# zhoujoey/ORB-SLAM3-Mac

Hardware: AMD Instinct MI355X
Metric: ORB extract+match frames/sec (higher is better)
Workload: dtype u8; 1 GPU; vga: synthetic 640x480 batch=1024 per GPU, 8-level pyramid, 1000 feats/frame, ORB extract + Hamming 2-NN match (Frame.cc:1146) + SearchForInitialization (ORBmatcher.cc:710) vs successor frame; pipelines=1, matchers=side by side (two contexts), frames_total=1024

## Files before the change

include/orbhip.h:

```cpp
#ifndef ORBHIP_H
#define ORBHIP_H
#include <stddef.h>
#include <stdint.h>
#ifdef __cplusplus
extern "C" {
#endif

#define ORBHIP_OK 0
#define ORBHIP_E_BADARG (-1)
#define ORBHIP_E_NODEVICE (-2)
#define ORBHIP_E_HIP (-3)
#define ORBHIP_E_CAPACITY (-4)
#define ORBHIP_E_ABORTED (-5)
#define ORBHIP_E_NOTSPD (-6)
#define ORBHIP_E_EMPTY (-7)

typedef struct {
    float x, y, size, angle, response;
    int32_t octave, class_id;
} orbhip_keypoint;

typedef struct orbhip_ctx orbhip_ctx;
typedef struct orbhip_extractor orbhip_extractor;

const char *orbhip_version(void);
const char *orbhip_last_error(void);

int orbhip_ctx_create(int device, void *stream, orbhip_ctx **out);
void orbhip_ctx_destroy(orbhip_ctx *ctx);
int orbhip_ctx_synchronize(orbhip_ctx *ctx);
int orbhip_ctx_wait_for(orbhip_ctx *ctx, orbhip_ctx *other);
int orbhip_ctx_check_status(orbhip_ctx *ctx);
void *orbhip_ctx_stream(orbhip_ctx *ctx);

int orbhip_extractor_create(orbhip_ctx *ctx, int nfeatures, float scale_factor, int nlevels,
                            int ini_th_fast, int min_th_fast, orbhip_extractor **out);
void orbhip_extractor_destroy(orbhip_extractor *ext);

int orbhip_extractor_levels(const orbhip_extractor *ext);
int orbhip_extractor_table(const orbhip_extractor *ext, int which, float *out);
int orbhip_extractor_features_per_level(const orbhip_extractor *ext, int *out);
int orbhip_extractor_umax(const orbhip_extractor *ext, int *out16);
int orbhip_blur_half_widths(int *out19);

int orbhip_extractor_reserve(orbhip_extractor *ext, int width, int height, int max_batch);
int orbhip_extractor_max_keypoints(const orbhip_extractor *ext);

int orbhip_extract_batch_device(orbhip_extractor *ext, const uint8_t *d_images, int width,
                                int height, size_t row_stride, size_t frame_stride, int batch,
                                int lap0, int lap1);
int orbhip_extractor_results(orbhip_extractor *ext, orbhip_keypoint **d_kp, uint8_t **d_desc,
                             int32_t **d_count, int32_t **d_mono_index);
int orbhip_extract_batch_host(orbhip_extractor *ext, const uint8_t *h_images, int width, int height,
                              size_t row_stride, size_t frame_stride, int batch, int lap0, int lap1,
                              orbhip_keypoint *kp_out, uint8_t *desc_out, int cap,
                              int32_t *count_out, int32_t *mono_out);
int orbhip_extract_batch_host_view(orbhip_extractor *ext, const uint8_t *h_images, int width, int height, size_t row_stride,
                                   size_t frame_stride, int batch, int lap0, int lap1, const orbhip_keypoint **kp_view,
                                   const uint8_t **desc_view, int *row_capacity, const int32_t **count_view, const int32_t **mono_view);
int orbhip_extractor_blur_kernel(const orbhip_extractor *ext, int batch);
int orbhip_extractor_fast_kernel(const orbhip_extractor *ext);
int orbhip_extractor_blur_tiled(const orbhip_extractor *ext, int batch);
int orbhip_extractor_desc_plan(const orbhip_extractor *ext, int batch, int32_t *kp_base, int32_t *kp_cap, int32_t *waves_per_xcd);

int orbhip_extractor_resize_band_rows(const orbhip_extractor *ext, int level);

int orbhip_extractor_last_frame(orbhip_extractor *ext, int frame, const orbhip_keypoint **d_kp, const uint8_t **d_desc,
                                const orbhip_keypoint **h_kp_view, const uint8_t **h_desc_view, int32_t *count, unsigned long long *generation);

int orbhip_extractor_level_dims(const orbhip_extractor *ext, int level, int *w, int *h);
int orbhip_extractor_get_pyramid_level(orbhip_extractor *ext, int frame, int level, int padded,
                                       uint8_t *h_out, size_t out_stride);
int orbhip_extractor_get_pyramid_padded(orbhip_extractor *ext, int frame, uint8_t *const *levels_out, const size_t *strides);
int orbhip_extractor_get_blurred_level(orbhip_extractor *ext, int frame, int level,
                                       uint8_t *h_out, size_t out_stride);
int orbhip_extractor_get_fast_candidates(orbhip_extractor *ext, int frame, int level,
                                         int32_t *xs, int32_t *ys, int32_t *scores, int cap,
                                         int32_t *n_out);
int orbhip_extractor_get_level_keypoints(orbhip_extractor *ext, int frame, int level,
                                         orbhip_keypoint *out, int cap, int32_t *n_out);

int orbhip_extractor_set_graph_mode(orbhip_extractor *ext, int enable);

#define ORBHIP_STAGE_PYRAMID 0
#define ORBHIP_STAGE_FAST_CELLS 1
#define ORBHIP_STAGE_BLUR 2
#define ORBHIP_STAGE_OCTREE 3
#define ORBHIP_STAGE_DESC 4
#define ORBHIP_STAGE_ASSEMBLE 5
#define ORBHIP_STAGE_COUNT 6
int orbhip_extractor_set_profiling(orbhip_extractor *ext, int enable);
int orbhip_extractor_stage_ms(orbhip_extractor *ext, float *ms_out );

int orbhip_descriptor_distance(const uint8_t *a32, const uint8_t *b32);

int orbhip_match_bf2nn_device(orbhip_ctx *ctx, const uint8_t *d_descA, const int32_t *d_nA,
                              size_t strideA, const uint8_t *d_descB, const int32_t *d_nB,
                              size_t strideB, int pairs, int max_n, double ratio,
                              int32_t *d_idx2, int32_t *d_dist2, uint8_t *d_accept);

int orbhip_search_for_initialization_device(orbhip_ctx *ctx,
        const orbhip_keypoint *d_kpA, const uint8_t *d_descA, const int32_t *d_nA,
        const orbhip_keypoint *d_kpB, const uint8_t *d_descB, const int32_t *d_nB,
        int pairs, int max_n, size_t frame_stride_kp , float min_x, float min_y,
        float max_x, float max_y, int window_size, float nn_ratio, int check_orientation,
        float *d_prev_matched, int32_t *d_matches12, int32_t *d_nmatches);

int orbhip_prev_matched_init_device(orbhip_ctx *ctx, const orbhip_keypoint *d_kp, size_t frame_stride_kp,
                                    int frames, int max_n, float *d_prev_matched);

typedef struct orbhip_proj_query {
    float u, v, radius, ur, angle;
    int32_t min_level, max_level, has_obs;
} orbhip_proj_query;
int orbhip_search_by_projection_device(orbhip_ctx *ctx, const orbhip_proj_query *d_q, const uint8_t *d_desc_q,
                                       const int32_t *d_nq, int max_q, const orbhip_keypoint *d_kp,
                                       const uint8_t *d_desc, const float *d_u_right, const int32_t *d_n, int max_n,
                                       size_t frame_stride_kp, int pairs, float min_x, float min_y, float max_x,
                                       float max_y, int th_high, int check_orientation, int32_t *d_train_match,
                                       int32_t *d_nmatches);

int orbhip_search_local_map_device(orbhip_ctx *ctx, const orbhip_proj_query *d_q, const uint8_t *d_desc_q,
                                   const int32_t *d_nq, int max_q, const orbhip_keypoint *d_kp,
                                   const uint8_t *d_desc, const float *d_u_right, const int32_t *d_n, int max_n,
                                   size_t frame_stride_kp, int pairs, float min_x, float min_y, float max_x,
                                   float max_y, int th_high, float nn_ratio, int32_t *d_train_match,
                                   int32_t *d_nmatches);

int orbhip_search_by_projection_rig_device(orbhip_ctx *ctx, int mode, const orbhip_proj_query *d_q, const uint8_t *d_desc_q,
                                           const int32_t *d_nq, int max_q, const orbhip_keypoint *d_kp, const uint8_t *d_desc,
                                           const int32_t *d_n, const int32_t *d_nleft, const int32_t *d_mirror, int max_n,
                                           size_t frame_stride_kp, int pairs, float min_x, float min_y, float max_x, float max_y,
                                           int th_high, float nn_ratio, int check_orientation, int32_t *d_train_match,
                                           int32_t *d_nmatches);

int orbhip_debug_sbp_handed_back(orbhip_ctx *ctx, int32_t *flags_out, int cap, int *pairs_out);

int orbhip_search_by_projection_host(orbhip_ctx *ctx, int mode, const orbhip_proj_query *q, const uint8_t *desc_q, int nq,
                                     const orbhip_keypoint *kp, const uint8_t *desc, const float *u_right, int n,
                                     float min_x, float min_y, float max_x, float max_y, int th_high, float nn_ratio,
                                     int check_orientation, int32_t *train_match_inout, int32_t *nmatches_out);
int orbhip_search_by_projection_rig_host(orbhip_ctx *ctx, int mode, const orbhip_proj_query *q, const uint8_t *desc_q, int nq,
                                         const orbhip_keypoint *kp, const uint8_t *desc, int n, int nleft, const int32_t *mirror,
                                         float min_x, float min_y, float max_x, float max_y, int th_high, float nn_ratio,
                                         int check_orientation, int32_t *train_match_inout, int32_t *nmatches_out);
int orbhip_search_for_initialization_host(orbhip_ctx *ctx, const orbhip_keypoint *kpA, const uint8_t *descA, int nA,
                                          const orbhip_keypoint *kpB, const uint8_t *descB, int nB, float min_x, float min_y,
                                          float max_x, float max_y, int window_size, float nn_ratio, int check_orientation,
                                          float *prev_matched_inout, int32_t *matches12_out, int32_t *nmatches_out);
int orbhip_search_by_projection_host_resident(orbhip_ctx *ctx, int mode, const orbhip_proj_query *q, const uint8_t *desc_q, int nq,
                                              const orbhip_keypoint *kp_host, const orbhip_keypoint *d_kp, const uint8_t *d_desc, const float *u_right, int n,
                                              float min_x, float min_y, float max_x, float max_y, int th_high, float nn_ratio,
                                              int check_orientation, int32_t *train_match_inout, int32_t *nmatches_out);
int orbhip_search_for_initialization_host_resident(orbhip_ctx *ctx, const orbhip_keypoint *kpA, const uint8_t *descA, int nA,
                                                   const orbhip_keypoint *kpB_host, const orbhip_keypoint *d_kpB, const uint8_t *d_descB, int nB, float min_x, float min_y,
                                                   float max_x, float max_y, int window_size, float nn_ratio, int check_orientation,
                                                   float *prev_matched_inout, int32_t *matches12_out, int32_t *nmatches_out);

int orbhip_fuse_search_device(orbhip_ctx *ctx, const orbhip_proj_query *d_q, const uint8_t *d_desc_q, const int32_t *d_nq,
                              int max_q, const orbhip_keypoint *d_kp, const uint8_t *d_desc, const float *d_u_right,
                              const int32_t *d_n, int max_n, size_t frame_stride_kp, int pairs,
                              const float *inv_level_sigma2, int nlevels, float min_x, float min_y, float max_x, float max_y,
                              int32_t *d_best_idx, int32_t *d_best_dist);

int orbhip_search_by_bow_device(orbhip_ctx *ctx,
        const int32_t *d_kf_node_ids, const int32_t *d_kf_node_start, const int32_t *d_kf_feat, const int32_t *d_kf_nnodes,
        const uint8_t *d_kf_valid, const orbhip_keypoint *d_kf_kp, const uint8_t *d_kf_desc,
        const int32_t *d_f_node_ids, const int32_t *d_f_node_start, const int32_t *d_f_feat, const int32_t *d_f_nnodes,
        const orbhip_keypoint *d_f_kp, const uint8_t *d_f_desc, const int32_t *d_nF,
        int pairs, int max_nodes, int max_n, size_t frame_stride_kp, float nn_ratio, int check_orientation,
        int32_t *d_match_f, int32_t *d_nmatches);

int orbhip_search_by_bow_rig_device(orbhip_ctx *ctx,
        const int32_t *d_kf_node_ids, const int32_t *d_kf_node_start, const int32_t *d_kf_feat, const int32_t *d_kf_nnodes,
        const uint8_t *d_kf_valid, const orbhip_keypoint *d_kf_kp, const uint8_t *d_kf_desc,
        const int32_t *d_f_node_ids, const int32_t *d_f_node_start, const int32_t *d_f_feat, const int32_t *d_f_nnodes,
        const orbhip_keypoint *d_f_kp, const uint8_t *d_f_desc, const int32_t *d_nF, const int32_t *d_nleft,
        int pairs, int max_nodes, int max_n, size_t frame_stride_kp, float nn_ratio, int check_orientation,
        int32_t *d_match_f, int32_t *d_nmatches);

int orbhip_search_by_bow_host(orbhip_ctx *ctx,
        const int32_t *kf_node_ids, const int32_t *kf_node_start, const int32_t *kf_feat, int kf_nnodes, const uint8_t *kf_valid,
        const orbhip_keypoint *kf_kp, const uint8_t *kf_desc, int nK,
        const int32_t *f_node_ids, const int32_t *f_node_start, const int32_t *f_feat, int f_nnodes,
        const orbhip_keypoint *f_kp, const uint8_t *f_desc, int nF, int nleft,
        float nn_ratio, int check_orientation, int32_t *match_f_out, int32_t *nmatches_out);
int orbhip_search_by_bow_host_resident(orbhip_ctx *ctx,
        const int32_t *kf_node_ids, const int32_t *kf_node_start, const int32_t *kf_feat, int kf_nnodes, const uint8_t *kf_valid,
        const orbhip_keypoint *kf_kp, const uint8_t *kf_desc, int nK,
        const int32_t *f_node_ids, const int32_t *f_node_start, const int32_t *f_feat, int f_nnodes,
        const orbhip_keypoint *f_kp_host, const orbhip_keypoint *d_f_kp, const uint8_t *d_f_desc, int nF,
        float nn_ratio, int check_orientation, int32_t *match_f_out, int32_t *nmatches_out);

int orbhip_search_by_bow_kf_device(orbhip_ctx *ctx,
        const int32_t *d_node_ids1, const int32_t *d_node_start1, const int32_t *d_feat1, const int32_t *d_nnodes1,
        const uint8_t *d_valid1, const orbhip_keypoint *d_kp1, const uint8_t *d_desc1, const int32_t *d_n1,
        const int32_t *d_node_ids2, const int32_t *d_node_start2, const int32_t *d_feat2, const int32_t *d_nnodes2,
        const uint8_t *d_valid2, const orbhip_keypoint *d_kp2, const uint8_t *d_desc2, const int32_t *d_n2,
        int pairs, int max_nodes, int max_n, size_t frame_stride_kp, float nn_ratio, int check_orientation,
        int32_t *d_matches12, int32_t *d_nmatches);

typedef struct orbhip_tri_pair { float F12[9]; float ep_x, ep_y; int32_t only_stereo, coarse; } orbhip_tri_pair;

int orbhip_search_for_triangulation_device(orbhip_ctx *ctx,
        const int32_t *d_nid1, const uint8_t *d_has_mp1, const orbhip_keypoint *d_kp1, const uint8_t *d_desc1, const float *d_u_right1,
        const int32_t *d_n1,
        const int32_t *d_node_ids2, const int32_t *d_node_start2, const int32_t *d_feat2, const int32_t *d_nnodes2,
        const uint8_t *d_has_mp2, const orbhip_keypoint *d_kp2, const uint8_t *d_desc2, const float *d_u_right2, const int32_t *d_n2,
        const orbhip_tri_pair *d_pair, int pairs, int max_nodes, int max_n, size_t frame_stride_kp,
        const float *scale_factors, const float *level_sigma2, int nlevels, int check_orientation,
        int32_t *d_matches12, int32_t *d_nmatches);

typedef struct orbhip_tri_pair_general {
    float R12[4][9], t12[4][3];
    float F12[4][9];
    float cam1[2][8], cam2[2][8];
    int32_t cam1_type[2], cam2_type[2];
    float ep_x, ep_y;
    int32_t nleft1, nleft2;
    int32_t only_stereo, coarse;
} orbhip_tri_pair_general;
int orbhip_search_for_triangulation_general_device(orbhip_ctx *ctx,
        const int32_t *d_nid1, const uint8_t *d_has_mp1, const orbhip_keypoint *d_kp1, const uint8_t *d_desc1, const float *d_u_right1,
        const int32_t *d_n1,
        const int32_t *d_node_ids2, const int32_t *d_node_start2, const int32_t *d_feat2, const int32_t *d_nnodes2,
        const uint8_t *d_has_mp2, const orbhip_keypoint *d_kp2, const uint8_t *d_desc2, const float *d_u_right2, const int32_t *d_n2,
        const orbhip_tri_pair_general *d_pair, int pairs, int max_nodes, int max_n, size_t frame_stride_kp,
        const float *level_sigma2_1, const float *scale_factors2, const float *level_sigma2_2, int nlevels, int check_orientation,
        int32_t *d_matches12, int32_t *d_nmatches);

typedef struct orbhip_tri_pair_poses { float Tcw1[2][12], Tcw2[2][12]; } orbhip_tri_pair_poses;
int orbhip_match_and_triangulate_device(orbhip_ctx *ctx,
        const int32_t *d_nid1, const uint8_t *d_has_mp1, const orbhip_keypoint *d_kp1, const uint8_t *d_desc1, const int32_t *d_n1,
        const int32_t *d_node_ids2, const int32_t *d_node_start2, const int32_t *d_feat2, const int32_t *d_nnodes2,
        const uint8_t *d_has_mp2, const orbhip_keypoint *d_kp2, const uint8_t *d_desc2, const int32_t *d_n2,
        const orbhip_tri_pair_general *d_pair, const orbhip_tri_pair_poses *d_poses, int pairs, int max_nodes, int max_n, size_t frame_stride_kp,
        const float *level_sigma2_1, const float *level_sigma2_2, int nlevels, int check_orientation,
        int32_t *d_matches12, float *d_points12, int32_t *d_nmatches);
int orbhip_match_and_triangulate_host(orbhip_ctx *ctx,
        const int32_t *nid1, const uint8_t *has_mp1, const orbhip_keypoint *kp1, const uint8_t *desc1, int n1,
        const int32_t *node_ids2, const int32_t *node_start2, const int32_t *feat2, int nnodes2,
        const uint8_t *has_mp2, const orbhip_keypoint *kp2, const uint8_t *desc2, int n2,
        const orbhip_tri_pair_general *pair, const orbhip_tri_pair_poses *poses, const float *level_sigma2_1, const float *level_sigma2_2,
        int nlevels, int check_orientation, int32_t *matches12_out, float *points12_out, int32_t *nmatches_out);

typedef struct orbhip_newpoints_pair {
    float cam1[2][8], cam2[2][8];
    int32_t cam1_type[2], cam2_type[2];
    int32_t nleft1, nleft2;
    float Tcw1[2][12], Tcw2[2][12];
    float Twc1[12], Twc2[12];
    float Ow1[2][3], Ow2[2][3];
    float mb1, mb2;
    float mbf;
    float ratio_factor;
    int32_t far_points;
    float th_far_points;
} orbhip_newpoints_pair;
int orbhip_create_new_map_points_device(orbhip_ctx *ctx,
        const orbhip_keypoint *d_kp1, const orbhip_keypoint *d_kp1_raw, const float *d_u_right1, const float *d_depth1, const int32_t *d_n1,
        const orbhip_keypoint *d_kp2, const orbhip_keypoint *d_kp2_raw, const float *d_u_right2, const float *d_depth2, const int32_t *d_n2,
        const int32_t *d_matches12, const orbhip_newpoints_pair *pair, int pairs, int max_n, size_t frame_stride_kp,
        const float *level_sigma2_1, const float *scale_factors1, const float *level_sigma2_2, const float *scale_factors2, int nlevels,
        uint8_t *d_has_mp1, uint8_t *d_has_mp2, float *d_x3D, uint8_t *d_outcome, int32_t *d_n_created);

typedef struct orbhip_newpoints_keyframe {
    const orbhip_keypoint *kp;
    const orbhip_keypoint *kp_raw;
    const uint8_t *desc;
    const float *u_right, *depth;
    const uint8_t *has_mp;
    int32_t n;
    const int32_t *nid;
    const int32_t *node_ids, *node_start, *feat;
    int32_t nnodes;
    const float *level_sigma2, *scale_factors;
} orbhip_newpoints_keyframe;
int orbhip_create_new_map_points_host(orbhip_ctx *ctx, const orbhip_newpoints_keyframe *cur, const orbhip_newpoints_keyframe *neigh,
        const orbhip_tri_pair_general *geom, const orbhip_newpoints_pair *pair, int n_neigh, int nlevels, int check_orientation,
        int32_t *matches12_out, float *x3D_out, uint8_t *outcome_out, int32_t *n_created_out, uint8_t *has_mp1_out);

int orbhip_search_for_triangulation_host(orbhip_ctx *ctx,
        const int32_t *nid1, const uint8_t *has_mp1, const orbhip_keypoint *kp1, const uint8_t *desc1, const float *u_right1, int n1,
        const int32_t *node_ids2, const int32_t *node_start2, const int32_t *feat2, int nnodes2,
        const uint8_t *has_mp2, const orbhip_keypoint *kp2, const uint8_t *desc2, const float *u_right2, int n2,
        const orbhip_tri_pair_general *pair, const float *level_sigma2_1, const float *scale_factors2, const float *level_sigma2_2,
        int nlevels, int check_orientation, int32_t *matches12_out, int32_t *nmatches_out);
int orbhip_fuse_search_host(orbhip_ctx *ctx, const orbhip_proj_query *q, const uint8_t *desc_q, int nq, const orbhip_keypoint *kp,
                            const uint8_t *desc, const float *u_right, int n, const float *inv_level_sigma2, int nlevels,
                            float min_x, float min_y, float max_x, float max_y, int32_t *best_idx_out, int32_t *best_dist_out);
int orbhip_search_by_bow_kf_host(orbhip_ctx *ctx,
        const int32_t *node_ids1, const int32_t *node_start1, const int32_t *feat1, int nnodes1, const uint8_t *valid1,
        const orbhip_keypoint *kp1, const uint8_t *desc1, int n1,
        const int32_t *node_ids2, const int32_t *node_start2, const int32_t *feat2, int nnodes2, const uint8_t *valid2,
        const orbhip_keypoint *kp2, const uint8_t *desc2, int n2,
        float nn_ratio, int check_orientation, int32_t *matches12_out, int32_t *nmatches_out);

int orbhip_undistort_keypoints_device(orbhip_ctx *ctx, const orbhip_keypoint *d_kp, const int32_t *d_n, int frames, int max_n,
                                      size_t frame_stride_kp, float fx, float fy, float cx, float cy, const float *dist_coef,
                                      int n_dist, orbhip_keypoint *d_kp_un);

int orbhip_assign_features_to_grid_device(orbhip_ctx *ctx, const orbhip_keypoint *d_kp, const int32_t *d_n, int frames, int max_n,
                                          size_t frame_stride_kp, float min_x, float min_y, float max_x, float max_y,
                                          int32_t *d_cell_start, int32_t *d_items);

int orbhip_assign_features_to_grid_rig_device(orbhip_ctx *ctx, const orbhip_keypoint *d_kp, const int32_t *d_n, const int32_t *d_nleft,
                                              int frames, int max_n, size_t frame_stride_kp, float min_x, float min_y, float max_x,
                                              float max_y, int32_t *d_cell_start, int32_t *d_items);

int orbhip_bow_vectors_device(orbhip_ctx *ctx, const int32_t *d_word_id, const double *d_weight, const int32_t *d_node_id,
                              const int32_t *d_n, int frames, int max_n, int max_nodes,
                              int32_t *d_node_ids, int32_t *d_node_start, int32_t *d_feat, int32_t *d_nnodes,
                              int32_t *d_bow_word, double *d_bow_value, int32_t *d_nwords);

int orbhip_distinctive_descriptors_device(orbhip_ctx *ctx, const uint8_t *d_desc, const int32_t *d_n, int points, int max_n,
                                          int32_t *d_best_idx, uint8_t *d_best_desc);

int orbhip_bow_transform_device(orbhip_ctx *ctx, const uint8_t *d_desc, const int32_t *d_n, int frames, int max_n,
                                size_t frame_stride, const uint8_t *d_node_desc, const int32_t *d_child_start,
                                const int32_t *d_child_ids, const int32_t *d_node_word, const double *d_node_weight,
                                int L, int levelsup, int32_t *d_word_id, double *d_weight, int32_t *d_nid);

int orbhip_compute_stereo_matches_device(orbhip_extractor *left, orbhip_extractor *right, float mb, float mbf,
                                         float *d_u_right, float *d_depth, int32_t *d_n_matches);

int orbhip_compute_stereo_matches_host(orbhip_extractor *left, orbhip_extractor *right, float mb, float mbf,
                                       float *u_right_out, float *depth_out, int n, int32_t *n_matches_out);

int orbhip_compute_stereo_fisheye_matches_device(orbhip_ctx *ctx,
        const orbhip_keypoint *d_kpL, const uint8_t *d_descL, const int32_t *d_nL, const int32_t *d_monoL, size_t strideL,
        const orbhip_keypoint *d_kpR, const uint8_t *d_descR, const int32_t *d_nR, const int32_t *d_monoR, size_t strideR,
        int batch, int max_n, int cam1_type, const float *cam1, int cam2_type, const float *cam2, const float *Rlr, const float *tlr,
        const float *level_sigma2, int nlevels,
        int32_t *d_l2r, int32_t *d_r2l, float *d_depth, float *d_x3d, int32_t *d_n_matches);

int orbhip_compute_stereo_fisheye_matches_host(orbhip_extractor *left, orbhip_extractor *right, int cam1_type, const float *cam1,
        int cam2_type, const float *cam2, const float *Rlr, const float *tlr, const float *level_sigma2, int nlevels,
        int32_t *l2r_out, float *depth_out, float *x3d_out, int n_left, int32_t *r2l_out, int n_right, int32_t *n_matches_out);

typedef struct {
    int32_t n_poses;
    int32_t n_points;
    int32_t n_edges;
    const uint8_t *pose_fixed;
    const int32_t *edge_pose;
    const int32_t *edge_point;
// ... 394 lines not shown
```

orb-slam3-mac_amd/csrc/fast_kernels.hip:

```cpp
#include "orb_internal.h"
#include "wave_dpp.h"
#include <algorithm>
#include <mutex>
#include <vector>
#include <cstdio>
#include <cstdlib>
#include <cstring>

typedef short s16x2 __attribute__((ext_vector_type(2)));
typedef uint32_t u32_unaligned __attribute__((aligned(1)));

__device__ __forceinline__ s16x2 as_s16x2(uint32_t v) { return __builtin_bit_cast(s16x2, v); }
__device__ __forceinline__ uint32_t as_u32(s16x2 v) { return __builtin_bit_cast(uint32_t, v); }
__device__ __forceinline__ s16x2 pkmin(s16x2 a, s16x2 b) { return __builtin_elementwise_min(a, b); }
__device__ __forceinline__ s16x2 pkmax(s16x2 a, s16x2 b) { return __builtin_elementwise_max(a, b); }
__device__ __forceinline__ s16x2 pkmin3(s16x2 a, s16x2 b, s16x2 c)
{
    uint32_t r;
    asm("v_pk_minimum3_f16 %0, %1, %2, %3" : "=v"(r) : "v"(as_u32(a)), "v"(as_u32(b)), "v"(as_u32(c)));
    return as_s16x2(r);
}
__device__ __forceinline__ s16x2 pkmax3(s16x2 a, s16x2 b, s16x2 c)
{
    uint32_t r;
    asm("v_pk_maximum3_f16 %0, %1, %2, %3" : "=v"(r) : "v"(as_u32(a)), "v"(as_u32(b)), "v"(as_u32(c)));
    return as_s16x2(r);
}
__device__ __forceinline__ s16x2 pair_odd(uint32_t hi, uint32_t lo) { return as_s16x2(__builtin_amdgcn_alignbit(hi, lo, 16)); }

template <int PITCH>
__device__ __forceinline__ s16x2 fc_compass(const uint32_t *q)
{
    const s16x2 v = as_s16x2(q[0]);
    const s16x2 n = as_s16x2(q[3 * PITCH]), s = as_s16x2(q[-3 * PITCH]);
    const s16x2 e = pair_odd(q[2], q[1]), w = pair_odd(q[-1], q[-2]);
    const s16x2 se = as_s16x2(q[2 * PITCH + 1]), nw = as_s16x2(q[-2 * PITCH - 1]);
    const s16x2 ne = as_s16x2(q[-2 * PITCH + 1]), sw = as_s16x2(q[2 * PITCH - 1]);
    const s16x2 lo = pkmax(pkmax3(pkmin(n, s), pkmin(e, w), pkmin(se, nw)), pkmin(ne, sw));
    const s16x2 hi = pkmin(pkmin3(pkmax(n, s), pkmax(e, w), pkmax(se, nw)), pkmax(ne, sw));
    return pkmax(v - lo, hi - v);
}

template <int PITCH>
__device__ __forceinline__ s16x2 fc_arc_score(const uint32_t *q)
{
    s16x2 p[16];
    {
        const uint32_t *r = q + 3 * PITCH;
        p[15] = pair_odd(r[0], r[-1]); p[0] = as_s16x2(r[0]); p[1] = pair_odd(r[1], r[0]);
        r = q + 2 * PITCH; p[14] = as_s16x2(r[-1]); p[2] = as_s16x2(r[1]);
        r = q + PITCH; p[13] = pair_odd(r[-1], r[-2]); p[3] = pair_odd(r[2], r[1]);
        p[12] = pair_odd(q[-1], q[-2]); p[4] = pair_odd(q[2], q[1]);
        r = q - PITCH; p[11] = pair_odd(r[-1], r[-2]); p[5] = pair_odd(r[2], r[1]);
        r = q - 2 * PITCH; p[10] = as_s16x2(r[-1]); p[6] = as_s16x2(r[1]);
        r = q - 3 * PITCH; p[9] = pair_odd(r[0], r[-1]); p[8] = as_s16x2(r[0]); p[7] = pair_odd(r[1], r[0]);
    }
    s16x2 lo2[8], hi2[8], lo4[8], hi4[8];
#pragma unroll
    for (int m = 0; m < 8; m++) { lo2[m] = pkmin(p[2 * m + 1], p[(2 * m + 2) & 15]); hi2[m] = pkmax(p[2 * m + 1], p[(2 * m + 2) & 15]); }
#pragma unroll
    for (int m = 0; m < 8; m++) { lo4[m] = pkmin(lo2[m], lo2[(m + 1) & 7]); hi4[m] = pkmax(hi2[m], hi2[(m + 1) & 7]); }
    s16x2 xl[8], xh[8];
#pragma unroll
    for (int m = 0; m < 8; m++) {
        const s16x2 e0 = p[2 * m], e1 = p[(2 * m + 9) & 15];
        xl[m] = pkmin3(lo4[m], lo4[(m + 2) & 7], pkmax(e0, e1));
        xh[m] = pkmax3(hi4[m], hi4[(m + 2) & 7], pkmin(e0, e1));
    }
    const s16x2 Lo = pkmax(pkmax3(pkmax3(xl[0], xl[1], xl[2]), xl[3], xl[4]), pkmax3(xl[5], xl[6], xl[7]));
    const s16x2 Hi = pkmin(pkmin3(pkmin3(xh[0], xh[1], xh[2]), xh[3], xh[4]), pkmin3(xh[5], xh[6], xh[7]));
    const s16x2 v = as_s16x2(q[0]);
    return pkmax(v - Hi, Lo - v);
}

#define FC_ID(by, bp) (((by) << 5) | (bp))
#define FC_U(v) as_s16x2(__builtin_amdgcn_perm(0u, (uint32_t)(v), 0x0c010c00u))
#define FC_STAGE(NCH_, NLD_) do { \
        const int last = (dh + 6) * NCH_ - 1; \
        _Pragma("unroll") \
        for (int t = 0; t < NLD_; t++) { \
            const int i = min(lane + 64 * t, last); \
            const int r = (int)(__umul24((uint32_t)i, 65536u / NCH_ + 1) >> 16), c = i - r * NCH_; \
            uint4 a, b; \
            a.x = __builtin_amdgcn_perm(0u, ld[t].x, 0x0c010c00u); a.y = __builtin_amdgcn_perm(0u, ld[t].x, 0x0c030c02u); \
            a.z = __builtin_amdgcn_perm(0u, ld[t].y, 0x0c010c00u); a.w = __builtin_amdgcn_perm(0u, ld[t].y, 0x0c030c02u); \
            b.x = __builtin_amdgcn_perm(0u, ld[t].z, 0x0c010c00u); b.y = __builtin_amdgcn_perm(0u, ld[t].z, 0x0c030c02u); \
            b.z = __builtin_amdgcn_perm(0u, ld[t].w, 0x0c010c00u); b.w = __builtin_amdgcn_perm(0u, ld[t].w, 0x0c030c02u); \
            uint4 *dst = reinterpret_cast<uint4 *>(&PT[r * PITCH + 8 * c]); \
            dst[0] = a; dst[1] = b; \
        } \
        uint4 *scz = reinterpret_cast<uint4 *>(SC); \
        for (int i = lane; i < ((dh + 2) * SPITCH + 7) / 8; i += 64) scz[i] = make_uint4(0u, 0u, 0u, 0u); \
    } while (0)
#define FC_NMS_NEIGHBOURS() \
    sc = q[0]; \
    const s16x2 V = pkmax(FC_U(q[-SPITCH]), FC_U(q[SPITCH])); \
    const s16x2 Lc = pkmax3(FC_U(q[-SPITCH - 1]), FC_U(q[-1]), FC_U(q[SPITCH - 1])); \
    const s16x2 Rc = pkmax3(FC_U(q[-SPITCH + 1]), FC_U(q[1]), FC_U(q[SPITCH + 1]))

struct FcCell {
    int frame, lvl, ci, cj;
    int dw, dh;
    int ipitch;
    const uint8_t *src;
    int ncols, nrows, wcell, hcell, cell_base, cell_cap, tpr, rpt;
};
#define FC_SGPR(x) __builtin_amdgcn_readfirstlane(x)
__device__ __forceinline__ void fc_cell_geom(const FastParams &P, FcCell &C)
{
    const FcLevel &L = P.lv[C.lvl];
    C.ncols = FC_SGPR(L.ncols); C.nrows = FC_SGPR(L.nrows); C.wcell = FC_SGPR(L.wcell); C.hcell = FC_SGPR(L.hcell);
    C.cell_base = FC_SGPR(L.cell_base); C.cell_cap = FC_SGPR(L.cell_cap); C.tpr = FC_SGPR(L.tpr); C.rpt = FC_SGPR(L.rpt);
    C.ipitch = FC_SGPR(L.img_pitch) & 0xFFFF;
    const int max_bx = FC_SGPR(L.max_bx), max_by = FC_SGPR(L.max_by);
    const int ini_y = ORB_MINB + C.ci * C.hcell, ini_x = ORB_MINB + C.cj * C.wcell;
    int max_y = ini_y + C.hcell + 6, max_x = ini_x + C.wcell + 6;
    C.src = L.img + (size_t)C.frame * L.frame_stride + (size_t)(ini_y * C.ipitch + ini_x - 1);
    C.dw = 0; C.dh = 0;
    if (ini_y >= max_by - 3 || ini_x >= max_bx - 6) return;
    if (max_y > max_by) max_y = max_by;
    if (max_x > max_bx) max_x = max_bx;
    C.dw = max_x - ini_x - 6; C.dh = max_y - ini_y - 6;
    if (C.dw <= 0 || C.dh <= 0) { C.dw = 0; C.dh = 0; }
}
template <int NCH, int NLD, typename CELL>
__device__ __forceinline__ void fc_issue_loads(const CELL &C, int lane, uint4 (&ld)[NLD])
{
    const int last = max((C.dh + 6) * NCH - 1, 0);
#pragma unroll
    for (int t = 0; t < NLD; t++) {
        const int i = min(lane + 64 * t, last);
        const int r = (int)(__umul24((uint32_t)i, 65536u / NCH + 1) >> 16), c = i - r * NCH;
        const u32x4_unaligned v = *reinterpret_cast<const u32x4_unaligned *>(C.src + (uint32_t)(__umul24((uint32_t)r, (uint32_t)C.ipitch) + 16u * (uint32_t)c));
        ld[t] = make_uint4(v.x, v.y, v.z, v.w);
    }
}

#ifdef FC_PROF
__device__ unsigned long long g_fc_prof[12];
extern "C" int orbhip_debug_fc_prof(unsigned long long *out8, int reset)
{
    if (out8 && hipMemcpyFromSymbol(out8, HIP_SYMBOL(g_fc_prof), 96) != hipSuccess) return -1;
    if (reset) { unsigned long long z[12] = {0}; if (hipMemcpyToSymbol(HIP_SYMBOL(g_fc_prof), z, 96) != hipSuccess) return -1; }
    return 0;
}
#define FC_T(i) do { const unsigned long long t_ = __builtin_readcyclecounter(); fc_acc[i] += t_ - fc_prev; fc_prev = t_; } while (0)
#else
#define FC_T(i) do { } while (0)
#endif
template <int NCH, int SPITCH, int NLD>
__global__ __launch_bounds__(64) void k_fast_cells(FastParams P)
{
    constexpr int PITCH = 8 * NCH;
    extern __shared__ __attribute__((aligned(16))) uint32_t fc_lds[];
    const int lane = threadIdx.x;
    uint32_t *PT = fc_lds;
    uint16_t *SC = reinterpret_cast<uint16_t *>(PT + P.rows * PITCH);
    uint16_t *Q = SC + (P.srows + 2) * SPITCH;
    const unsigned lid = xcd_logical_id(blockIdx.x, gridDim.x);
    const int lvl_lo = FC_SGPR(P.lvl_lo), lvl_hi = FC_SGPR(P.lvl_hi);
    const int cell_lo = FC_SGPR(P.lv[lvl_lo].cell_base);
    const int cps = (lvl_hi < P.nlevels ? FC_SGPR(P.lv[lvl_hi].cell_base) : FC_SGPR(P.cells_per_frame)) - cell_lo;
    const long total_cells = (long)P.batch * cps;
    const int chunk = FC_SGPR(P.chunk);
    const long nchunks = (total_cells + chunk - 1) / chunk;
    if ((long)lid >= nchunks) return;
    const int nlevels = lvl_hi, ini_th = FC_SGPR(P.ini_th), min_th = FC_SGPR(P.min_th), cpf = FC_SGPR(P.cells_per_frame);
    auto decode = [&](long gi, FcCell &X) {
        X.frame = (int)(gi / cps);
        const int cell = cell_lo + (int)(gi - (long)X.frame * cps);
        X.lvl = lvl_lo;
        for (int l = lvl_lo + 1; l < nlevels; l++) if (cell >= P.lv[l].cell_base) X.lvl = l;
        const int c = cell - P.lv[X.lvl].cell_base;
        X.ci = c / P.lv[X.lvl].ncols; X.cj = c - X.ci * P.lv[X.lvl].ncols;
        X.frame = FC_SGPR(X.frame); X.lvl = FC_SGPR(X.lvl); X.ci = FC_SGPR(X.ci); X.cj = FC_SGPR(X.cj);
        fc_cell_geom(P, X);
    };
    long ch = lid;
    long g = ch * chunk, g_end = min(g + chunk, total_cells);
    FcCell C;
    decode(g, C);
    uint4 ld[NLD];
    fc_issue_loads<NCH, NLD>(C, lane, ld);
    const int lo_th = min(ini_th, min_th);
#ifdef FC_PROF
    unsigned long long fc_acc[12] = {0, 0, 0, 0, 0, 0, 0, 0, 0, 0, 0, 0}, fc_prev = __builtin_readcyclecounter();
    const unsigned long long fc_t0 = fc_prev;
#endif
    for (bool more = true; more;) {
        const int dw = C.dw, dh = C.dh;
        const int npb = (dw + 1) >> 1;
        const int cell = C.cell_base + C.ci * C.ncols + C.cj;
        uint32_t *cnt_out = P.cell_count + (size_t)C.frame * cpf + cell;
        uint32_t *list = P.cell_list + (size_t)C.frame * P.cell_list_frame_stride + (size_t)cell * C.cell_cap;
        const int key_x0 = 3 + C.cj * C.wcell, key_y0 = 3 + C.ci * C.hcell;
        const int cell_cap = C.cell_cap, tpr = C.tpr, rptT = C.rpt;
#ifdef FC_PROF
        __builtin_amdgcn_s_waitcnt(0x0F70);
        FC_T(11);
#endif
        if (dw > 0) FC_STAGE(NCH, NLD);
        FC_T(8);
        FcCell N = C;
        g++;
        if (g < g_end) {
            N.cj++;
            if (N.cj == C.ncols) { N.cj = 0; N.ci++; }
            if (N.ci == C.nrows) { N.ci = 0; N.lvl++; }
            if (N.lvl == nlevels) { N.lvl = lvl_lo; N.frame++; }
            fc_cell_geom(P, N);
        } else {
            ch += gridDim.x;
            more = ch < nchunks;
            if (more) { g = ch * chunk; g_end = min(g + chunk, total_cells); decode(g, N); }
        }
        FC_T(9);
        if (more) fc_issue_loads<NCH, NLD>(N, lane, ld);
        FC_T(10);
        if (dw <= 0) { if (lane == 0) *cnt_out = 0; C = N; continue; }
        FC_T(0);
        wave_lds_sync();
        const int tr0 = (int)(__umul24((uint32_t)lane, P.div_magic[tpr]) >> 16), tg = lane - tr0 * tpr;
        const bool lane_rows = tr0 < rptT && 2 * tg < npb, pair1 = 2 * tg + 1 < npb;
        int total = 0;
        FC_T(1);
        for (int pass = 0; pass < 2; pass++) {
            const int th = pass == 0 ? ini_th : min_th;
            const s16x2 thP = (s16x2){(short)(th + 1), (short)(th + 1)};
            int nq1 = 0;
            for (int y0 = 0; y0 < dh; y0 += rptT) {
                const int by = y0 + tr0;
                bool f0 = false, f1 = false;
                if (lane_rows && by < dh) {
                    const uint32_t *q = &PT[(by + 3) * PITCH + 2 * tg + 2];
                    const uint32_t SIGN = 0x80008000u;
                    const s16x2 M0 = fc_compass<PITCH>(q), M1 = fc_compass<PITCH>(q + 1);
                    f0 = (as_u32(M0 - thP) & SIGN) != SIGN;
                    f1 = ((as_u32(M1 - thP) & SIGN) != SIGN) & pair1;
                }
                const unsigned long long b0 = __ballot(f0), b1 = __ballot(f1);
                const int pos = nq1 + (int)__builtin_amdgcn_mbcnt_hi((uint32_t)(b0 >> 32), __builtin_amdgcn_mbcnt_lo((uint32_t)b0, 0u)) +
                                (int)__builtin_amdgcn_mbcnt_hi((uint32_t)(b1 >> 32), __builtin_amdgcn_mbcnt_lo((uint32_t)b1, 0u));
                if (f0) Q[pos] = (uint16_t)FC_ID(by, 2 * tg);
                if (f1) Q[pos + (f0 ? 1 : 0)] = (uint16_t)FC_ID(by, 2 * tg + 1);
                nq1 += __popcll(b0) + __popcll(b1);
            }
            wave_lds_sync();
            FC_T(2);
            for (int i0 = 0; i0 < nq1; i0 += 64) {
                const int i = min(i0 + lane, nq1 - 1);
                const int id = Q[i], by = id >> 5, bp = id & 31;
                const s16x2 S = fc_arc_score<PITCH>(&PT[(by + 3) * PITCH + bp + 2]);
                if (i0 + lane < nq1) {
                    const uint32_t lo = S.x > lo_th ? (uint32_t)(S.x - 1) : 0u;
                    const uint32_t hi = (S.y > lo_th && 2 * bp + 1 < dw) ? (uint32_t)(S.y - 1) : 0u;
                    SC[(by + 1) * SPITCH + bp + 1] = (uint16_t)(lo | (hi << 8));
                }
            }
            wave_lds_sync();
            FC_T(3);
            for (int i0 = 0; i0 < nq1; i0 += 64) {
                const int i = i0 + lane;
                uint32_t keep = 0, sc = 0;
                int by = 0, bp = 0;
                if (i < nq1) {
                    const int id = Q[i];
                    by = id >> 5; bp = id & 31;
                    const uint16_t *q = &SC[(by + 1) * SPITCH + bp + 1];
                    FC_NMS_NEIGHBOURS();
                    const int sl = (int)(sc & 0xFFu), sr = (int)(sc >> 8);
                    const int nbl = max(max((int)V.x, (int)V.y), max((int)Lc.y, sr));
                    const int nbr = max(max((int)V.x, (int)V.y), max((int)Rc.x, sl));
                    if (sl >= th && sl > nbl) keep |= 1u;
                    if (sr >= th && sr > nbr) keep |= 2u;
                }
                const int mine = __popc(keep);
                const int inc = wave_incl_scan(mine);
                int offs = total + inc - mine;
                if (keep & 1u) { if (offs < cell_cap) list[offs] = ORB_PACK_KEY(2 * bp + key_x0, by + key_y0, sc & 0xFFu); offs++; }
                if (keep & 2u) { if (offs < cell_cap) list[offs] = ORB_PACK_KEY(2 * bp + 1 + key_x0, by + key_y0, (sc >> 8) & 0xFFu); }
                total += __builtin_amdgcn_readlane(inc, 63);
            }
            FC_T(4);
            if (total > 0 || min_th == ini_th) break;
            wave_lds_sync();
        }
        if (total > cell_cap) { if (lane == 0) atomicExch(P.status, ORBHIP_E_CAPACITY); total = cell_cap; }
        if (lane == 0) *cnt_out = (uint32_t)total;
        C = N;
        FC_T(5);
#ifdef FC_PROF
        fc_acc[6]++;
#endif
    }
#ifdef FC_PROF
    fc_acc[7] = __builtin_readcyclecounter() - fc_t0;
    if (lane == 0) for (int i = 0; i < 12; i++) atomicAdd(&g_fc_prof[i], fc_acc[i]);
#endif
}

#define FR_PITCH 40
#define FR_SPITCH 40
#define FR_NCH 5
struct FrRun {
    int frame, lvl, ci, cj, nc;
    int dw0, dw1, dh;
    int ipitch; const uint8_t *src;
    int ncols, nrows, wcell, hcell, cell_base, cell_cap, rpc, rpr;
};
__device__ __forceinline__ void fr_run_geom(const FastParams &P, FrRun &C)
{
    const FcLevel &L = P.lv[C.lvl];
    C.ncols = FC_SGPR(L.ncols); C.nrows = FC_SGPR(L.nrows); C.wcell = FC_SGPR(L.wcell); C.hcell = FC_SGPR(L.hcell);
    C.cell_base = FC_SGPR(L.cell_base); C.cell_cap = FC_SGPR(L.cell_cap); C.rpc = FC_SGPR(L.rpc); C.rpr = FC_SGPR(L.rpr);
    C.ipitch = FC_SGPR(L.img_pitch) & 0xFFFF;
    C.nc = min(C.rpc, C.ncols - C.cj);
    const int max_bx = FC_SGPR(L.max_bx), max_by = FC_SGPR(L.max_by);
    const int ini_y = ORB_MINB + C.ci * C.hcell, ini_x = ORB_MINB + C.cj * C.wcell;
    C.src = L.img + (size_t)C.frame * L.frame_stride + (size_t)(ini_y * C.ipitch + ini_x - 1);
    C.dw0 = 0; C.dw1 = 0; C.dh = 0;
    if (ini_y >= max_by - 3) return;
    C.dh = min(ini_y + C.hcell + 6, max_by) - ini_y - 6;
    if (C.dh <= 0) { C.dh = 0; return; }
    if (ini_x < max_bx - 6) C.dw0 = max(min(ini_x + C.wcell + 6, max_bx) - ini_x - 6, 0);
    const int ini_x1 = ini_x + C.wcell;
    if (C.nc > 1 && ini_x1 < max_bx - 6) C.dw1 = max(min(ini_x1 + C.wcell + 6, max_bx) - ini_x1 - 6, 0);
    if (C.dw0 == 0) C.dw1 = 0;
}

template <int FR_NLD>
__global__ __launch_bounds__(64) void k_fast_runs(FastParams P)
{
    constexpr int PITCH = FR_PITCH, SPITCH = FR_SPITCH;
    extern __shared__ __attribute__((aligned(16))) uint32_t fc_lds[];
    const int lane = threadIdx.x;
    uint32_t *PT = fc_lds;
    uint16_t *SC = reinterpret_cast<uint16_t *>(PT + P.run_rows * PITCH);
    uint16_t *Q = SC + (P.srows + 2) * SPITCH;
    const int q0cap = FC_SGPR(P.run_q0);
    const unsigned lid = xcd_logical_id(blockIdx.x, gridDim.x);
    const int lvl_lo = FC_SGPR(P.lvl_lo), lvl_hi = FC_SGPR(P.lvl_hi);
    const int run_lo = FC_SGPR(P.lv[lvl_lo].run_base);
    const int rps = (lvl_hi < P.nlevels ? FC_SGPR(P.lv[lvl_hi].run_base) : FC_SGPR(P.runs_per_frame)) - run_lo;
    const long total_runs = (long)P.batch * rps;
    const int chunk = FC_SGPR(P.chunk);
    const long nchunks = (total_runs + chunk - 1) / chunk;
    if ((long)lid >= nchunks) return;
    const int nlevels = lvl_hi, ini_th = FC_SGPR(P.ini_th), min_th = FC_SGPR(P.min_th), cpf = FC_SGPR(P.cells_per_frame);
    auto decode = [&](long gi, FrRun &X) {
        X.frame = (int)(gi / rps);
        const int run = run_lo + (int)(gi - (long)X.frame * rps);
        X.lvl = lvl_lo;
        for (int l = lvl_lo + 1; l < nlevels; l++) if (run >= P.lv[l].run_base) X.lvl = l;
        const int r = run - P.lv[X.lvl].run_base;
        X.ci = r / P.lv[X.lvl].rpr; X.cj = (r - X.ci * P.lv[X.lvl].rpr) * P.lv[X.lvl].rpc;
        X.frame = FC_SGPR(X.frame); X.lvl = FC_SGPR(X.lvl); X.ci = FC_SGPR(X.ci); X.cj = FC_SGPR(X.cj);
        fr_run_geom(P, X);
    };
    long ch = lid;
    long g = ch * chunk, g_end = min(g + chunk, total_runs);
    FrRun C;
    decode(g, C);
    uint4 ld[FR_NLD];
    fc_issue_loads<FR_NCH, FR_NLD>(C, lane, ld);
    const int lo_th = min(ini_th, min_th);
    const int bp = lane & 31, half = lane >> 5;
    for (bool more = true; more;) {
        const int dw0 = C.dw0, dw1 = C.dw1, dw = dw0 + dw1, dh = C.dh;
        const int npb = (dw + 1) >> 1;
        const int cell = C.cell_base + C.ci * C.ncols + C.cj;
        uint32_t *cnt_out = P.cell_count + (size_t)C.frame * cpf + cell;
        uint32_t *list = P.cell_list + (size_t)C.frame * P.cell_list_frame_stride + (size_t)cell * C.cell_cap;
        const int key_x0 = 3 + C.cj * C.wcell, key_y0 = 3 + C.ci * C.hcell;
        const int cell_cap = C.cell_cap, nc = C.nc;
        if (dw > 0) FC_STAGE(FR_NCH, FR_NLD);
        FrRun N = C;
        g++;
        if (g < g_end) {
            N.cj += C.rpc;
            if (N.cj >= C.ncols) { N.cj = 0; N.ci++; }
            if (N.ci == C.nrows) { N.ci = 0; N.lvl++; }
            if (N.lvl == nlevels) { N.lvl = lvl_lo; N.frame++; }
            fr_run_geom(P, N);
        } else {
            ch += gridDim.x;
            more = ch < nchunks;
            if (more) { g = ch * chunk; g_end = min(g + chunk, total_runs); decode(g, N); }
        }
        if (more) fc_issue_loads<FR_NCH, FR_NLD>(N, lane, ld);
        if (dw <= 0) { if (lane < nc) cnt_out[lane] = 0; C = N; continue; }
        wave_lds_sync();
        const int B = dw1 > 0 ? dw0 : (1 << 20);
        const int hh = (dh + 1) >> 1;
        const int rb = half * hh;
        const int rows_mine = min(hh, dh - rb);
        int tot0 = 0, tot1 = 0;
        uint32_t empty = 0;
        for (int pass = 0; pass < 2; pass++) {
            const int th = pass == 0 ? ini_th : min_th;
            const s16x2 thP = (s16x2){(short)(th + 1), (short)(th + 1)};
            bool col_on = bp < npb;
            if (pass) col_on = col_on && ((((2 * bp >= B) ? 2u : 1u) | ((2 * bp + 1 >= B) ? 2u : 1u)) & empty) != 0;
            int nq0 = 0, nq1 = 0;
            {
                const uint32_t *col = PT + rb * PITCH + bp + 1;
                const int rows_on = col_on ? rows_mine : 0;
                uint32_t rm[13], rc[13], rp[13];
#pragma unroll
                for (int i = 0; i < 6; i++) { rm[i] = col[i * PITCH]; rc[i] = col[i * PITCH + 1]; rp[i] = col[i * PITCH + 2]; }
                const uint32_t SIGN = 0x80008000u;
                for (int y0 = 0; y0 < hh; y0 += 7) {
                    const uint32_t *cy = col + y0 * PITCH;
                    uint32_t cm2[7], cp2[7];
#pragma unroll
                    for (int i = 0; i < 7; i++) {
                        rm[6 + i] = cy[(6 + i) * PITCH]; rc[6 + i] = cy[(6 + i) * PITCH + 1]; rp[6 + i] = cy[(6 + i) * PITCH + 2];
                        cm2[i] = cy[(3 + i) * PITCH - 1]; cp2[i] = cy[(3 + i) * PITCH + 3];
                    }
                    bool f[7];
#pragma unroll
                    for (int i = 0; i < 7; i++) {
                        const s16x2 v = as_s16x2(rc[i + 3]);
                        const s16x2 n = as_s16x2(rc[i + 6]), so = as_s16x2(rc[i]);
                        const s16x2 e = pair_odd(cp2[i], rp[i + 3]), w = pair_odd(rm[i + 3], cm2[i]);
                        const s16x2 se = as_s16x2(rp[i + 5]), nw = as_s16x2(rm[i + 1]);
                        const s16x2 ne = as_s16x2(rp[i + 1]), sw = as_s16x2(rm[i + 5]);
                        const s16x2 lo = pkmax(pkmax3(pkmin(n, so), pkmin(e, w), pkmin(se, nw)), pkmin(ne, sw));
                        const s16x2 hi = pkmin(pkmin3(pkmax(n, so), pkmax(e, w), pkmax(se, nw)), pkmax(ne, sw));
                        const s16x2 M = pkmax(v - lo, hi - v);
                        f[i] = y0 + i < rows_on && (as_u32(M - thP) & SIGN) != SIGN;
                    }
#pragma unroll
                    for (int i = 0; i < 7; i++) {
                        const unsigned long long b = __ballot(f[i]);
                        const uint32_t blo = (uint32_t)b, bhi = (uint32_t)(b >> 32);
                        const int m = (int)__builtin_amdgcn_mbcnt_hi(bhi, __builtin_amdgcn_mbcnt_lo(blo, 0u));
                        const int pos = m + (half ? q0cap + nq1 - __popc(blo) : nq0);
                        if (f[i]) Q[pos] = (uint16_t)FC_ID(rb + y0 + i, bp);
                        nq0 += __popc(blo); nq1 += __popc(bhi);
                    }
#pragma unroll
                    for (int i = 0; i < 6; i++) { rm[i] = rm[7 + i]; rc[i] = rc[7 + i]; rp[i] = rp[7 + i]; }
                }
            }
            const int nq = nq0 + nq1;
            wave_lds_sync();
            for (int i0 = 0; i0 < nq; i0 += 64) {
                const int i = min(i0 + lane, nq - 1);
                const int id = Q[i < nq0 ? i : q0cap + i - nq0], by = id >> 5, qp = id & 31;
                const s16x2 S = fc_arc_score<PITCH>(&PT[(by + 3) * PITCH + qp + 2]);
                if (i0 + lane < nq) {
                    const uint32_t lo = S.x > lo_th ? (uint32_t)(S.x - 1) : 0u;
                    const uint32_t hi = (S.y > lo_th && 2 * qp + 1 < dw) ? (uint32_t)(S.y - 1) : 0u;
                    SC[(by + 1) * SPITCH + qp + 1] = (uint16_t)(lo | (hi << 8));
                }
            }
            wave_lds_sync();
            for (int i0 = 0; i0 < nq; i0 += 64) {
                const int i = i0 + lane;
                uint32_t keep = 0, sc = 0;
                int by = 0, qp = 0;
                if (i < nq) {
                    const int id = Q[i < nq0 ? i : q0cap + i - nq0];
                    by = id >> 5; qp = id & 31;
                    const uint16_t *q = &SC[(by + 1) * SPITCH + qp + 1];
                    FC_NMS_NEIGHBOURS();
                    const int xl = 2 * qp, xr = xl + 1;
                    const int sl = (int)(sc & 0xFFu), sr = (int)(sc >> 8);
                    const int nbl = max(max((int)V.x, xl != B ? (int)Lc.y : 0), xr != B ? max((int)V.y, sr) : 0);
                    const int nbr = max(max((int)V.y, xr + 1 != B ? (int)Rc.x : 0), xr != B ? max((int)V.x, sl) : 0);
                    const bool onL = !pass || ((xl >= B ? 2u : 1u) & empty), onR = !pass || ((xr >= B ? 2u : 1u) & empty);
                    if (sl >= th && sl > nbl && onL) keep |= 1u;
                    if (sr >= th && sr > nbr && onR) keep |= 2u;
                }
                const int xl = 2 * qp;
                const bool kL = keep & 1u, kR = keep & 2u, cL = xl >= B, cR = xl + 1 >= B;
#pragma unroll
                for (int c = 0; c < 2; c++) {
                    const bool mL = kL && (int)cL == c, mR = kR && (int)cR == c;
                    const unsigned long long bL = __ballot(mL), bR = __ballot(mR);
                    const int before = (int)__builtin_amdgcn_mbcnt_hi((uint32_t)(bL >> 32), __builtin_amdgcn_mbcnt_lo((uint32_t)bL, 0u)) +
                                       (int)__builtin_amdgcn_mbcnt_hi((uint32_t)(bR >> 32), __builtin_amdgcn_mbcnt_lo((uint32_t)bR, 0u));
                    const int base = c ? tot1 : tot0;
                    uint32_t *lst = list + (size_t)c * cell_cap;
                    if (mL) { const int o = base + before; if (o < cell_cap) lst[o] = ORB_PACK_KEY(xl + key_x0, by + key_y0, sc & 0xFFu); }
                    if (mR) { const int o = base + before + (mL ? 1 : 0); if (o < cell_cap) lst[o] = ORB_PACK_KEY(xl + 1 + key_x0, by + key_y0, (sc >> 8) & 0xFFu); }
                    const int add = __popcll(bL) + __popcll(bR);
                    if (c) tot1 += add; else tot0 += add;
                }
            }
            if (pass || min_th == ini_th) break;
            empty = (tot0 == 0 && dw0 > 0 ? 1u : 0u) | (tot1 == 0 && dw1 > 0 ? 2u : 0u);
            if (!empty) break;
            wave_lds_sync();
        }
        if (tot0 > cell_cap || tot1 > cell_cap) { if (lane == 0) atomicExch(P.status, ORBHIP_E_CAPACITY); tot0 = min(tot0, cell_cap); tot1 = min(tot1, cell_cap); }
        if (lane == 0) { cnt_out[0] = (uint32_t)tot0; if (nc > 1) cnt_out[1] = (uint32_t)tot1; }
        C = N;
    }
}
const void *orb_fast_runs_func(int nld) { return nld == 4 ? reinterpret_cast<const void *>(k_fast_runs<4>) : reinterpret_cast<const void *>(k_fast_runs<6>); }

int orb_fast_runs_nld(const FastParams &F) { return (F.run_rows - 7) * FR_NCH <= 256 ? 4 : 6; }
int orb_fast_variant(const FastParams &F) { return F.use_runs ? (orb_fast_runs_nld(F) == 4 ? 2 : 3) : F.small_cells ? 1 : 0; }
void orb_plan_fast(const OrbParams &P, FastParams &F)
{
    memset(&F, 0, sizeof(F));
    int mw = 0, mh = 0;
    bool small = true;
    for (int l = 0; l < P.nlevels; l++) {
        const OrbLevel &L = P.lv[l];
        FcLevel &f = F.lv[l];
        mw = std::max(mw, L.wcell); mh = std::max(mh, L.hcell);
        f.max_bx = L.w - ORB_MINB; f.max_by = L.h - ORB_MINB;
        f.ncols = L.ncols; f.nrows = L.nrows; f.wcell = L.wcell; f.hcell = L.hcell; f.cell_base = L.cell_base; f.cell_cap = L.cell_cap;
        const int npb = (L.wcell + 1) >> 1;
        f.tpr = (npb + 1) >> 1; f.rpt = 64 / f.tpr;
        small = small && npb + 4 <= 24 && npb + 2 <= 24 && (L.hcell + 6) * 3 <= 64 * 2;
    }
    {
        int runs = 0;
        bool ok = true;
        for (int l = 0; l < P.nlevels; l++) {
            const OrbLevel &L = P.lv[l];
            FcLevel &f = F.lv[l];
            f.rpc = 2 * L.wcell <= 64 ? 2 : 1;
            f.rpr = (L.ncols + f.rpc - 1) / f.rpc;
            f.run_base = runs; runs += f.rpr * L.nrows;
            ok = ok && L.wcell <= 64 && L.hcell + 6 <= 70 && L.wcell >= 8 && L.hcell >= 8;
        }
        const int hh = (mh + 1) / 2;
        F.runs_per_frame = runs;
        F.run_rows = mh + 6 + 7;
        F.run_q0 = (hh * 32 + 7) & ~7;
        F.run_dw = F.run_rows * FR_PITCH + (((mh + 2) * FR_SPITCH + 2 * F.run_q0) + 1) / 2;
        F.run_dw = (F.run_dw + 3) & ~3;
        F.use_runs = ok && getenv("ORBHIP_FAST_KERNEL") && !strcmp(getenv("ORBHIP_FAST_KERNEL"), "runs") ? 1 : 0;
    }
    const int npb = (mw + 1) >> 1;
    F.small_cells = small ? 1 : 0;
    F.rows = mh + 6; F.srows = mh; F.qcap = (mh * npb + 1) & ~1;
    F.wave_dw = F.rows * (small ? 24 : 40) + ((F.srows + 2) * (small ? 24 : 32) + F.qcap + 1) / 2;
    F.wave_dw = (F.wave_dw + 3) & ~3;
    F.nlevels = P.nlevels; F.ini_th = P.ini_th; F.min_th = P.min_th; F.cells_per_frame = P.cells_per_frame;
    for (int n = 1; n < 34; n++) F.div_magic[n] = (uint32_t)(65536 / n + 1);
}

void orb_launch_fast_cells(const FastParams &F_, hipStream_t s, int max_per_cu, int lvl_lo, int lvl_hi)
{
    FastParams F = F_;
    F.lvl_lo = lvl_lo; F.lvl_hi = lvl_hi < 0 ? F.nlevels : lvl_hi;
    if (F.lvl_lo >= F.lvl_hi) return;
    const bool runs = F.use_runs != 0;
    const size_t lds = sizeof(uint32_t) * (size_t)(runs ? F.run_dw : F.wave_dw);
    const int nld = orb_fast_runs_nld(F);
    const int v = orb_fast_variant(F);
    int per_cu;
    {
        struct Occ { int dev, v, n; size_t lds; };
        static std::mutex occ_mu; static std::vector<Occ> occ_tab;
        int dev = 0; (void)hipGetDevice(&dev);
        std::lock_guard<std::mutex> g(occ_mu);
        const Occ *hit = nullptr;
        for (const Occ &o : occ_tab) if (o.dev == dev && o.v == v && o.lds == lds) { hit = &o; break; }
        if (!hit) {
            int n = 0;
            if (hipOccupancyMaxActiveBlocksPerMultiprocessor(&n, v >= 2 ? orb_fast_runs_func(nld) : orb_fast_cells_func(v), 64, lds) != hipSuccess || n < 1) n = (int)((160 * 1024) / (lds + 512));
            occ_tab.push_back(Occ{dev, v, n < 1 ? 1 : n, lds}); hit = &occ_tab.back();
            if (getenv("ORBHIP_DEBUG_FAST")) fprintf(stderr, "[orbhip] %s: %zu B of LDS per wave, %d waves per CU resident\n", v >= 2 ? "k_fast_runs" : "k_fast_cells", lds, hit->n);
        }
        per_cu = hit->n;
    }
    if (max_per_cu > 0 && per_cu > max_per_cu) per_cu = max_per_cu;
    long nblocks = (long)(F.n_cus > 0 ? F.n_cus : 256) * per_cu;
    const long total = runs ? (long)F.batch * ((F.lvl_hi < F.nlevels ? F.lv[F.lvl_hi].run_base : F.runs_per_frame) - F.lv[F.lvl_lo].run_base)
                            : (long)F.batch * ((F.lvl_hi < F.nlevels ? F.lv[F.lvl_hi].cell_base : F.cells_per_frame) - F.lv[F.lvl_lo].cell_base);
    if (nblocks > total) nblocks = (total + 7) / 8 * 8;
    static const int chunk_env = getenv("ORBHIP_TUNE_FAST_CHUNK") ? atoi(getenv("ORBHIP_TUNE_FAST_CHUNK")) : 0;
    const long fair = total / (8 * nblocks);
    const int cmax = runs ? 8 : 4;
    F.chunk = chunk_env > 0 ? chunk_env : (int)(fair < 1 ? 1 : fair > cmax ? cmax : fair);
    if (runs && nld == 4) hipLaunchKernelGGL(k_fast_runs<4>, dim3((unsigned)nblocks), dim3(64), lds, s, F);
    else if (runs) hipLaunchKernelGGL(k_fast_runs<6>, dim3((unsigned)nblocks), dim3(64), lds, s, F);
    else if (F.small_cells) hipLaunchKernelGGL((k_fast_cells<3, 24, 2>), dim3((unsigned)nblocks), dim3(64), lds, s, F);
    else hipLaunchKernelGGL((k_fast_cells<5, 32, 5>), dim3((unsigned)nblocks), dim3(64), lds, s, F);
}
const void *orb_fast_cells_func(int small) { return small ? reinterpret_cast<const void *>(k_fast_cells<3, 24, 2>) : reinterpret_cast<const void *>(k_fast_cells<5, 32, 5>); }
```

orb-slam3-mac_amd/csrc/orb_internal.h:

```cpp
#pragma once
#include <hip/hip_runtime.h>
#include <stdint.h>
#include <vector>
#include "../../include/orbhip.h"

#define ORB_MAX_LEVELS 16
#define ORB_EDGE 19
#define ORB_MINB 16
#define ORB_HALF_PATCH 15
#define ORB_RS_STEPS 24

struct OrbLevel {
    uint8_t *img;
    uint8_t *blur;
    size_t img_frame_stride;
    size_t blur_frame_stride;
    int w, h, img_pitch, blur_pitch;
    int blur_tiles_x;
    int ncols, nrows, wcell, hcell;
    int cell_base;
    int cell_cap;
    int quota;
    int key_base, key_cap;
    int kp_base, kp_cap;
    int n_ini;
    float hx;
    float scale;
    float size;
    const int16_t *xofs; const int16_t *xalpha; const int16_t *yofs; const int16_t *ybeta;
    const uint32_t *xchunk; const uint32_t *ytab;
    int resize_mode;
    int rs_rows;
};

struct OrbParams {
    OrbLevel lv[ORB_MAX_LEVELS];
    int nlevels, batch;
    int n_cus;
    int ini_th, min_th;
    int cells_per_frame;
    int keys_per_frame;
    int kps_per_frame;
    int max_kp;
    int oct_nc;
    int oct_dmax;
    int rows_min_batch;
    int bm_min_batch;
    int br_blocks[ORB_MAX_LEVELS + 1];
    int bs_tiles[ORB_MAX_LEVELS + 1];
    int desc_blocks_cap;
    int lap0, lap1;
    uint32_t *cell_count;
    uint32_t *cell_list;
    size_t cell_list_frame_stride;
    uint32_t *keys;
    uint16_t *node_of;
    uint32_t *lvl_kp;
#define ORB_PERM_MIN_BATCH 16
    uint16_t *lvl_perm;
    uint32_t *lvl_wkey;
    float *lvl_angle;
    uint8_t *lvl_desc;
    int32_t *lvl_count;
    int32_t *lvl_ncand;
    int32_t *status;
    orbhip_keypoint *out_kp;
    uint8_t *out_desc;
    int32_t *out_count;
    int32_t *out_mono;
    int umax[ORB_HALF_PATCH + 1];
    int gauss_q8[7];
    const uint4 *bm_th;
    const uint4 *bm_tv;
    int bm_cols[ORB_MAX_LEVELS + 1];
    int bm_init;
    int blur_tiled_ok;
    int blur_tiled;
    int blur_hw[ORB_EDGE];
};

struct FcLevel {
    const uint8_t *img; size_t frame_stride; int img_pitch;
    int max_bx, max_by;
    int ncols, nrows, wcell, hcell, cell_base, cell_cap;
    int tpr, rpt;
    int rpc, rpr, run_base;
};
struct FastParams {
    FcLevel lv[ORB_MAX_LEVELS];
    int nlevels, batch, ini_th, min_th, cells_per_frame;
    int n_cus;
    int chunk;
    int lvl_lo, lvl_hi;
    uint32_t *cell_count, *cell_list; size_t cell_list_frame_stride; int32_t *status;
    int rows, srows, qcap, wave_dw, small_cells;
    uint32_t div_magic[34];
    int runs_per_frame, run_rows, run_q0, run_dw, use_runs;
};

#define ORB_BLUR_TILE_OFF(x, y, tiles_x) ((((uint32_t)((y) >> 3) * (uint32_t)(tiles_x) + (uint32_t)((x) >> 4)) << 7) + (uint32_t)(((y) & 7) << 4) + (uint32_t)((x) & 15))
#define ORB_PACK_KEY(x, y, s) ((uint32_t)(x) | ((uint32_t)(y) << 12) | ((uint32_t)(s) << 24))
#define ORB_KEY_X(k) ((int)((k) & 0xFFFu))
#define ORB_KEY_Y(k) ((int)(((k) >> 12) & 0xFFFu))
#define ORB_KEY_S(k) ((int)((k) >> 24))

typedef uint32_t rs_u32x3 __attribute__((ext_vector_type(3)));
typedef rs_u32x3 rs_u32x3_a4 __attribute__((aligned(4)));
struct __attribute__((packed, aligned(1))) u32x4_unaligned { uint32_t x, y, z, w; };

__device__ __forceinline__ int hamming256(const uint4 &a0, const uint4 &a1, const uint4 &b0, const uint4 &b1)
{
    return __popc(a0.x ^ b0.x) + __popc(a0.y ^ b0.y) + __popc(a0.z ^ b0.z) + __popc(a0.w ^ b0.w) +
           __popc(a1.x ^ b1.x) + __popc(a1.y ^ b1.y) + __popc(a1.z ^ b1.z) + __popc(a1.w ^ b1.w);
}

struct StereoLevel {
    const uint8_t *imgL, *imgR;
    size_t fsL, fsR;
    int pitchL, pitchR, wR, pad_;
    float scale, inv_scale;
};
struct StereoArgs {
    StereoLevel lv[ORB_MAX_LEVELS];
    int nlevels, batch, max_kp, rows0;
    const orbhip_keypoint *kpL, *kpR;
    const uint8_t *descL, *descR;
    const int32_t *nL, *nR;
    float mb, mbf;
    float *u_right, *depth;
    int32_t *sad, *n_kept;
};
void orb_launch_stereo(const StereoArgs &A, hipStream_t s);

int orb_lds_optin(const void *func, int device, size_t need);

void orb_plan_fast(const OrbParams &P, FastParams &F);
bool orb_plan_resize(OrbParams &P, int level, const std::vector<int16_t> &xofs, const std::vector<int16_t> &xalpha, const std::vector<int16_t> &yofs,
                     const std::vector<int16_t> &ybeta, std::vector<uint32_t> &xchunk, std::vector<uint32_t> &ytab);
bool orb_plan_blur(OrbParams &P, std::vector<int8_t> &bm_th, std::vector<int8_t> &bm_tv);
int orb_blur_kernel(const OrbParams &P, int batch);

void orb_launch_resize(const OrbParams &P, int level, hipStream_t s);
void orb_launch_fast_cells(const FastParams &F, hipStream_t s, int max_per_cu, int lvl_lo = 0, int lvl_hi = -1);
const void *orb_fast_runs_func(int nld);
int orb_fast_runs_nld(const FastParams &F);
int orb_fast_variant(const FastParams &F);
const void *orb_fast_cells_func(int small);
#define ORB_OVERLAP_MIN_BATCH 16
#ifndef BLR_R
#define BLR_R 24
#endif
void orb_launch_blur(const OrbParams &P, hipStream_t s, int wgs_per_cu, int frame0 = 0, int nframes = -1);
void orb_launch_orient_desc(const OrbParams &P, hipStream_t s);
int orb_orient_desc_blocks(const OrbParams &P);
void orb_launch_octree(const OrbParams &P, hipStream_t s, int parts = 3);
void orb_launch_assemble(const OrbParams &P, hipStream_t s);
size_t orb_octree_lds_bytes(int nc);
int orb_octree_nc(const OrbParams &P);
int orb_octree_dmax(const OrbParams &P);
const void *orb_octree_func(int which = 0);
```

orb-slam3-mac_amd/csrc/orbhip_api.hip:

```cpp
#include "orb_internal.h"
#include "ctx_internal.h"
#include <cmath>
#include <cfloat>
#include <cstdio>
#include <cstdlib>
#include <cstring>
#include <string>
#include <vector>
#include <mutex>
#include <set>
#include <utility>

static thread_local std::string g_last_error;
extern "C" const char *orbhip_last_error(void) { return g_last_error.c_str(); }
extern "C" const char *orbhip_version(void) { return "orbhip 0.1 (gfx950)"; }

#define HIP_TRY(expr)                                                                   \
    do {                                                                                \
        hipError_t _e = (expr);                                                         \
        if (_e != hipSuccess) {                                                         \
            g_last_error = std::string(#expr) + ": " + hipGetErrorString(_e);           \
            return ORBHIP_E_HIP;                                                        \
        }                                                                               \
    } while (0)
// ... 79 lines not shown
    if (bytes <= c->pinned_bytes) return c->pinned;
    (void)hipStreamSynchronize(c->stream);
    if (c->pinned) (void)hipHostFree(c->pinned);
    c->pinned = nullptr; c->pinned_bytes = 0;
    const size_t want = std::max<size_t>(bytes + bytes / 2, 1 << 20);
    if (hipHostMalloc(&c->pinned, want, hipHostMallocDefault) != hipSuccess) { g_last_error = "hipHostMalloc(pinned staging arena)"; return nullptr; }
    c->pinned_bytes = want;
    return c->pinned;
}
void *orbhip_ctx_ba_arena_acquire_internal(orbhip_ctx *c, size_t bytes)
{
    if (c->ba_arena_busy) return nullptr;
    if (bytes > c->ba_arena_bytes) {
        (void)hipStreamSynchronize(c->stream);
        if (c->ba_arena) (void)hipFree(c->ba_arena);
        c->ba_arena = nullptr; c->ba_arena_bytes = 0;
        const size_t want = bytes + bytes / 4;
        if (hipMalloc(&c->ba_arena, want) != hipSuccess) return nullptr;
        c->ba_arena_bytes = want;
    }
    c->ba_arena_busy = true;
    return c->ba_arena;
}
void orbhip_ctx_ba_arena_release_internal(orbhip_ctx *c) { c->ba_arena_busy = false; }
int *orbhip_ctx_pinned_word_internal(orbhip_ctx *c)
{
    if (!c->pinned_word && hipHostMalloc((void **)&c->pinned_word, 256, hipHostMallocDefault) != hipSuccess) c->pinned_word = nullptr;
    return c->pinned_word;
}
void *orbhip_ctx_work_internal(orbhip_ctx *c, size_t bytes)
{
    if (bytes <= c->work_bytes) return c->work;
    (void)hipStreamSynchronize(c->stream);
    if (c->work) (void)hipFree(c->work);
    c->work = nullptr; c->work_bytes = 0;
    const size_t want = std::max<size_t>(bytes + bytes / 4, 1 << 20);
    if (hipMalloc(&c->work, want) != hipSuccess) { g_last_error = "hipMalloc(work arena)"; return nullptr; }
    c->work_bytes = want;
    return c->work;
}
void orbhip_set_last_error_internal(const char *msg) { g_last_error = msg; }
void orbhip_ctx_note_sbp_redo_internal(orbhip_ctx *c, size_t offset, int pairs) { c->sbp_redo_off = offset; c->sbp_redo_pairs = pairs; }
extern "C" int orbhip_debug_sbp_handed_back(orbhip_ctx *c, int32_t *flags_out, int cap, int *pairs_out)
{
    if (!c || !pairs_out || cap < 0 || (cap > 0 && !flags_out)) return ORBHIP_E_BADARG;
    HIP_TRY(hipStreamSynchronize(c->stream));
    *pairs_out = c->sbp_redo_pairs;
    const int m = c->sbp_redo_pairs < cap ? c->sbp_redo_pairs : cap;
    if (m > 0) {
        if (!c->work || c->sbp_redo_off + sizeof(int32_t) * (size_t)m > c->work_bytes) return ORBHIP_E_BADARG;
        HIP_TRY(hipMemcpy(flags_out, (const uint8_t *)c->work + c->sbp_redo_off, sizeof(int32_t) * (size_t)m, hipMemcpyDeviceToHost));
    }
    return ORBHIP_OK;
}
extern "C" int orbhip_ctx_check_status(orbhip_ctx *c)
{
    if (!c) return ORBHIP_E_BADARG;
    int32_t st = 0;
    HIP_TRY(hipStreamSynchronize(c->stream));
    HIP_TRY(hipMemcpy(&st, orbhip_ctx_status_internal(c), sizeof(st), hipMemcpyDeviceToHost));
    if (st) { HIP_TRY(hipMemset(orbhip_ctx_status_internal(c), 0, sizeof(int32_t))); g_last_error = "device-side capacity exceeded in a matcher kernel"; }
    return st;
}
int32_t *orbhip_ctx_status_internal(orbhip_ctx *c) { return c->status_redirect ? c->status_redirect : c->d_status; }
void orbhip_ctx_redirect_status_internal(orbhip_ctx *c, int32_t *p) { c->status_redirect = p; }
extern "C" void orbhip_ctx_destroy(orbhip_ctx *c)
{
    if (!c) return;
    (void)hipFree(c->d_status);
    if (c->scratch) (void)hipFree(c->scratch);
    if (c->work) (void)hipFree(c->work);
    if (c->pinned) (void)hipHostFree(c->pinned);
    if (c->ba_arena) (void)hipFree(c->ba_arena);
    if (c->pinned_word) (void)hipHostFree(c->pinned_word);
    if (c->own_stream) (void)hipStreamDestroy(c->stream);
    delete c;
}
extern "C" int orbhip_ctx_synchronize(orbhip_ctx *c)
{
    if (!c) return ORBHIP_E_BADARG;
    HIP_TRY(hipStreamSynchronize(c->stream));
    return ORBHIP_OK;
}
extern "C" int orbhip_ctx_wait_for(orbhip_ctx *c, orbhip_ctx *other)
{
    if (!c || !other) return ORBHIP_E_BADARG;
    if (c == other || c->stream == other->stream) return ORBHIP_OK;
    if (c->device != other->device) { g_last_error = "orbhip_ctx_wait_for: contexts of two devices"; return ORBHIP_E_BADARG; }
    HIP_TRY(hipSetDevice(c->device));
    hipEvent_t ev;
    HIP_TRY(hipEventCreateWithFlags(&ev, hipEventDisableTiming));
    HIP_TRY(hipEventRecord(ev, other->stream));
    HIP_TRY(hipStreamWaitEvent(c->stream, ev, 0));
    HIP_TRY(hipEventDestroy(ev));
    return ORBHIP_OK;
}
extern "C" void *orbhip_ctx_stream(orbhip_ctx *c) { return c ? (void *)c->stream : nullptr; }
hipStream_t orbhip_ctx_stream_internal(orbhip_ctx *c) { return c->stream; }
int orbhip_ctx_device_internal(orbhip_ctx *c) { return c->device; }
int orbhip_ctx_cus_internal(orbhip_ctx *c) { return c->n_cus; }
int orbhip_ctx_ba_schur_mode_internal(orbhip_ctx *c) { return c->ba_schur_mode; }
extern "C" int orbhip_ctx_set_ba_schur_mode(orbhip_ctx *c, int mode)
{
    if (!c || mode < 0 || mode > 2) return ORBHIP_E_BADARG;
    c->ba_schur_mode = mode;
    return ORBHIP_OK;
}

static inline int cv_round_f(float v) { return (int)lrintf(v); }
static inline int cv_round_d(double v) { return (int)lrint(v); }
static inline int align_up(int v, int a) { return (v + a - 1) / a * a; }

#define ORBHIP_PROF_SLOTS 32
struct orbhip_extractor {
    orbhip_ctx *ctx;
    int nfeatures, nlevels, ini_th, min_th;
    float scale_factor;
    float scale[ORB_MAX_LEVELS], inv_scale[ORB_MAX_LEVELS], sigma2[ORB_MAX_LEVELS], inv_sigma2[ORB_MAX_LEVELS];
    int per_level[ORB_MAX_LEVELS];
    int umax[ORB_HALF_PATCH + 1];
    int gauss_q8[7];
    int width, height, max_batch;
    bool level0_owned;
    OrbParams P;
    FastParams F;
    std::vector<void *> allocs;
    size_t bytes_reserved;
    int last_batch;
    bool profiling;
    hipEvent_t ev[ORBHIP_PROF_SLOTS][ORBHIP_STAGE_COUNT + 1];
    int ev_calls;
    bool ev_created;
    float stage_ms[ORBHIP_STAGE_COUNT];
    uint8_t *d_level0;
    int32_t *d_stereo_sad;
    bool graph_mode, graph_valid;
    hipStream_t aux; hipEvent_t ev_fork, ev_join, ev_pyr; bool aux_ok; int overlap;
    hipGraphExec_t graph_exec;
    int g_w, g_h, g_batch, g_lap0, g_lap1;
    size_t level0_frame_stride; int level0_pitch;
    uint8_t *d_outblob; size_t outblob_bytes, ob_kp, ob_desc;
    uint8_t *h_out; uint8_t *h_in; size_t h_in_bytes; int32_t *h_status;
    uint8_t *h_pyr; size_t h_pyr_bytes;
    unsigned long long generation, view_generation;
    int oct_dmax_tab;
};

extern "C" int orbhip_extractor_create(orbhip_ctx *ctx, int nfeatures, float scale_factor, int nlevels,
                                       int ini_th, int min_th, orbhip_extractor **out)
{
    if (!ctx || !out || nlevels < 1 || nlevels > ORB_MAX_LEVELS || nfeatures < 1 || !(scale_factor > 1.0f) || scale_factor > 2.0f)
        return ORBHIP_E_BADARG;
    orbhip_extractor *e = new orbhip_extractor();
    e->ctx = ctx; e->nfeatures = nfeatures; e->nlevels = nlevels; e->ini_th = ini_th; e->min_th = min_th;
    e->scale_factor = scale_factor;
    e->width = e->height = e->max_batch = 0; e->bytes_reserved = 0; e->last_batch = 0;
    e->profiling = false; e->ev_created = false; e->ev_calls = 0; e->d_level0 = nullptr; e->level0_owned = false;
    e->d_stereo_sad = nullptr;
    e->graph_mode = false; e->graph_valid = false; e->graph_exec = nullptr;
    e->aux = nullptr; e->ev_fork = e->ev_join = e->ev_pyr = nullptr; e->aux_ok = false; e->overlap = 1;
    e->d_outblob = nullptr; e->outblob_bytes = e->ob_kp = e->ob_desc = 0; e->h_out = e->h_in = e->h_pyr = nullptr; e->h_in_bytes = e->h_pyr_bytes = 0; e->h_status = nullptr;
    e->generation = 0; e->view_generation = ~0ull;
    memset(&e->P, 0, sizeof(e->P));
    memset(e->stage_ms, 0, sizeof(e->stage_ms));
    e->scale[0] = 1.0f; e->sigma2[0] = 1.0f;
    for (int i = 1; i < nlevels; i++) { e->scale[i] = e->scale[i - 1] * scale_factor; e->sigma2[i] = e->scale[i] * e->scale[i]; }
    for (int i = 0; i < nlevels; i++) { e->inv_scale[i] = 1.0f / e->scale[i]; e->inv_sigma2[i] = 1.0f / e->sigma2[i]; }
    float factor = 1.0f / scale_factor;
    float desired = nfeatures * (1 - factor) / (1 - (float)pow((double)factor, (double)nlevels));
    int sum = 0;
    for (int l = 0; l < nlevels - 1; l++) { e->per_level[l] = cv_round_f(desired); sum += e->per_level[l]; desired *= factor; }
    e->per_level[nlevels - 1] = std::max(nfeatures - sum, 0);
    int v, v0, vmax = (int)floor(ORB_HALF_PATCH * sqrtf(2.f) / 2 + 1), vmin = (int)ceil(ORB_HALF_PATCH * sqrtf(2.f) / 2);
    const double hp2 = ORB_HALF_PATCH * ORB_HALF_PATCH;
    for (v = 0; v <= vmax; ++v) e->umax[v] = cv_round_d(sqrt(hp2 - v * v));
    for (v = ORB_HALF_PATCH, v0 = 0; v >= vmin; --v) { while (e->umax[v0] == e->umax[v0 + 1]) ++v0; e->umax[v] = v0; ++v0; }
    {
        float cf[7]; double s = 0;
        for (int i = 0; i < 7; i++) { double x = i - 3.0; cf[i] = (float)exp(-0.5 / 4.0 * x * x); s += cf[i]; }
        s = 1. / s;
        for (int i = 0; i < 7; i++) { cf[i] = (float)(cf[i] * s); e->gauss_q8[i] = cv_round_f(cf[i] * 256.f); }
    }
    *out = e;
    return ORBHIP_OK;
}

static void ext_free_all(orbhip_extractor *e)
{
    for (void *p : e->allocs) (void)hipFree(p);
    e->allocs.clear();
    e->bytes_reserved = 0; e->width = e->height = e->max_batch = 0; e->d_level0 = nullptr; e->d_stereo_sad = nullptr;
    if (e->h_out) (void)hipHostFree(e->h_out);
    if (e->h_in) (void)hipHostFree(e->h_in);
    if (e->h_pyr) (void)hipHostFree(e->h_pyr);
    if (e->h_status) (void)hipHostFree(e->h_status);
    e->h_out = e->h_in = e->h_pyr = nullptr; e->h_status = nullptr; e->h_in_bytes = e->h_pyr_bytes = 0; e->d_outblob = nullptr; e->view_generation = ~0ull;
    if (e->graph_valid) { (void)hipGraphExecDestroy(e->graph_exec); e->graph_valid = false; }
}
static void ext_free_aux(orbhip_extractor *e)
{
    if (!e->aux_ok) return;
    (void)hipStreamSynchronize(e->aux);
    (void)hipEventDestroy(e->ev_fork); (void)hipEventDestroy(e->ev_join); (void)hipEventDestroy(e->ev_pyr); (void)hipStreamDestroy(e->aux);
    e->aux_ok = false;
}

extern "C" void orbhip_extractor_destroy(orbhip_extractor *e)
{
    if (!e) return;
    (void)hipStreamSynchronize(e->ctx->stream);
    ext_free_aux(e);
    ext_free_all(e);
    if (e->ev_created) for (auto &slot : e->ev) for (auto &ev : slot) (void)hipEventDestroy(ev);
    delete e;
}

extern "C" int orbhip_extractor_levels(const orbhip_extractor *e) { return e ? e->nlevels : ORBHIP_E_BADARG; }
extern "C" int orbhip_extractor_table(const orbhip_extractor *e, int which, float *out)
{
    if (!e || !out || which < 0 || which > 3) return ORBHIP_E_BADARG;
    const float *t = which == 0 ? e->scale : which == 1 ? e->inv_scale : which == 2 ? e->sigma2 : e->inv_sigma2;
    memcpy(out, t, sizeof(float) * e->nlevels);
    return ORBHIP_OK;
}
extern "C" int orbhip_extractor_features_per_level(const orbhip_extractor *e, int *out)
{
    if (!e || !out) return ORBHIP_E_BADARG;
    memcpy(out, e->per_level, sizeof(int) * e->nlevels);
    return ORBHIP_OK;
}
extern "C" int orbhip_extractor_umax(const orbhip_extractor *e, int *out16)
{
    if (!e || !out16) return ORBHIP_E_BADARG;
    memcpy(out16, e->umax, sizeof(int) * 16);
    return ORBHIP_OK;
}
extern "C" int orbhip_extractor_max_keypoints(const orbhip_extractor *e) { return e ? e->P.max_kp : ORBHIP_E_BADARG; }

template <typename T>
static int dev_alloc(orbhip_extractor *e, T **p, size_t count)
{
    void *q = nullptr;
    size_t bytes = std::max<size_t>(count * sizeof(T), 256);
    hipError_t err = hipMalloc(&q, bytes);
    if (err != hipSuccess) { g_last_error = std::string("hipMalloc: ") + hipGetErrorString(err); return ORBHIP_E_HIP; }
    e->allocs.push_back(q);
    e->bytes_reserved += bytes;
    *p = (T *)q;
    return ORBHIP_OK;
}

static void resize_tables(int sn, int dn, bool horizontal, std::vector<int16_t> &ofs, std::vector<int16_t> &coef)
{
    double scale = 1. / ((double)dn / sn);
    ofs.resize(dn); coef.resize(2 * dn);
    for (int d = 0; d < dn; d++) {
        float f = (float)((d + 0.5) * scale - 0.5);
        int s = (int)floorf(f);
        f -= s;
        if (horizontal) {
            if (s < 0) { f = 0; s = 0; }
            if (s >= sn - 1) { f = 0; s = sn - 1; }
        }
        int c0 = cv_round_f((1.f - f) * 2048), c1 = cv_round_f(f * 2048);
        ofs[d] = (int16_t)std::min(std::max(s, -32768), 32767);
        coef[2 * d] = (int16_t)std::min(std::max(c0, -32768), 32767);
        coef[2 * d + 1] = (int16_t)std::min(std::max(c1, -32768), 32767);
    }
}

extern "C" int orbhip_blur_half_widths(int *out19)
{
    if (!out19) return ORBHIP_E_BADARG;
    static const int8_t pat[1024] = {
#include "orb_pattern.inc"
    };
    double R2 = 0;
    for (int i = 0; i < 512; i++) R2 = std::max(R2, (double)pat[2 * i] * pat[2 * i] + (double)pat[2 * i + 1] * pat[2 * i + 1]);
    for (int d = 0; d < ORB_EDGE; d++) {
        const double t = std::max(d - 0.5, 0.0), q = R2 - t * t;
        out19[d] = q > 0 ? std::min((int)floor(sqrt(q) + 0.5), 18) : -64;
    }
    return ORBHIP_OK;
}

extern "C" int orbhip_extractor_reserve(orbhip_extractor *e, int width, int height, int max_batch)
{
    if (!e || width <= 0 || height <= 0 || max_batch <= 0) return ORBHIP_E_BADARG;
    if (e->width == width && e->height == height && e->max_batch >= max_batch) return ORBHIP_OK;
    if (width > 4096 + 2 * ORB_MINB || height > 4096 + 2 * ORB_MINB) { g_last_error = "image larger than 12-bit key packing"; return ORBHIP_E_BADARG; }
    HIP_TRY(hipSetDevice(e->ctx->device));
    HIP_TRY(hipStreamSynchronize(e->ctx->stream));
    ext_free_all(e);
    OrbParams &P = e->P;
    memset(&P, 0, sizeof(P));
    P.nlevels = e->nlevels; P.ini_th = e->ini_th; P.min_th = e->min_th;
    memcpy(P.umax, e->umax, sizeof(P.umax));
    memcpy(P.gauss_q8, e->gauss_q8, sizeof(P.gauss_q8));
    int cells = 0, keys = 0, kps = 0, max_cell_cap = 0;
    for (int l = 0; l < e->nlevels; l++) {
        OrbLevel &L = P.lv[l];
        L.w = cv_round_f((float)width * e->inv_scale[l]);
        L.h = cv_round_f((float)height * e->inv_scale[l]);
        const float w_ = (float)((L.w - ORB_EDGE + 3) - ORB_MINB), h_ = (float)((L.h - ORB_EDGE + 3) - ORB_MINB);
        if (w_ < 30.f || h_ < 30.f) { g_last_error = "pyramid level smaller than one FAST cell"; return ORBHIP_E_BADARG; }
        L.ncols = (int)(w_ / 30.f); L.nrows = (int)(h_ / 30.f);
        L.wcell = (int)ceilf(w_ / L.ncols); L.hcell = (int)ceilf(h_ / L.nrows);
        if (L.wcell + 6 > 64 || L.hcell + 6 > 64) { g_last_error = "FAST cell exceeds the 64x64 LDS tile"; return ORBHIP_E_BADARG; }
        max_cell_cap = std::max(max_cell_cap, ((L.wcell + 1) / 2) * ((L.hcell + 1) / 2));
        L.cell_base = cells; cells += L.ncols * L.nrows;
        L.quota = e->per_level[l];
        const int maxx = L.w - ORB_MINB, maxy = L.h - ORB_MINB;
        L.n_ini = (int)roundf((float)(maxx - ORB_MINB) / (maxy - ORB_MINB));
        if (L.n_ini < 1) { g_last_error = "nIni == 0 (image taller than 2x its width): undefined in the reference"; return ORBHIP_E_BADARG; }
        L.hx = (float)(maxx - ORB_MINB) / L.n_ini;
        L.scale = e->scale[l];
        L.size = (float)(int)(31 * e->scale[l]);
        L.kp_base = kps; L.kp_cap = align_up(std::max(L.quota + 8, 4 * L.n_ini + 4), 4); kps += L.kp_cap;
    }
    for (int l = 0; l < e->nlevels; l++) {
        OrbLevel &L = P.lv[l];
        L.cell_cap = max_cell_cap;
        L.key_base = keys;
        L.key_cap = std::min(L.ncols * L.nrows * max_cell_cap, ((L.w - 2 * ORB_MINB + 1) / 2 + L.ncols) * ((L.h - 2 * ORB_MINB + 1) / 2 + L.nrows));
        L.key_cap = std::min(L.key_cap, 0xFFFFF);
        keys += align_up(L.key_cap, 4);
    }
    P.cells_per_frame = cells; P.keys_per_frame = keys; P.kps_per_frame = kps; P.max_kp = align_up(kps, 8);
    orb_plan_fast(P, e->F);
    P.rows_min_batch = getenv("ORBHIP_ROWS_MIN_BATCH") ? atoi(getenv("ORBHIP_ROWS_MIN_BATCH")) : 16;
    std::vector<int8_t> bm_th, bm_tv;
    const bool bm_ok = orb_plan_blur(P, bm_th, bm_tv);
    P.cell_list_frame_stride = (size_t)cells * max_cell_cap;
    int rc;
    const size_t B = (size_t)max_batch;
    for (int l = 0; l < e->nlevels; l++) {
        OrbLevel &L = P.lv[l];
        L.img_pitch = align_up(L.w, 64); L.blur_pitch = L.img_pitch;
        L.img_frame_stride = (size_t)L.img_pitch * L.h;
        L.blur_tiles_x = (L.w + 15) / 16;
        L.blur_frame_stride = align_up(std::max((size_t)L.blur_pitch * L.h, (size_t)L.blur_tiles_x * ((L.h + 7) / 8) * 128), (size_t)128);
        if ((rc = dev_alloc(e, &L.img, B * L.img_frame_stride + 64))) return rc;
        if ((rc = dev_alloc(e, &L.blur, B * L.blur_frame_stride + 64))) return rc;
        if (l > 0) {
            std::vector<int16_t> xo, xa, yo, yb;
            resize_tables(P.lv[l - 1].w, L.w, true, xo, xa);
            resize_tables(P.lv[l - 1].h, L.h, false, yo, yb);
            int16_t *dxo, *dxa, *dyo, *dyb;
            if ((rc = dev_alloc(e, &dxo, xo.size()))) return rc;
            if ((rc = dev_alloc(e, &dxa, xa.size()))) return rc;
            if ((rc = dev_alloc(e, &dyo, yo.size()))) return rc;
            if ((rc = dev_alloc(e, &dyb, yb.size()))) return rc;
            HIP_TRY(hipMemcpy(dxo, xo.data(), xo.size() * 2, hipMemcpyHostToDevice));
            HIP_TRY(hipMemcpy(dxa, xa.data(), xa.size() * 2, hipMemcpyHostToDevice));
            HIP_TRY(hipMemcpy(dyo, yo.data(), yo.size() * 2, hipMemcpyHostToDevice));
            HIP_TRY(hipMemcpy(dyb, yb.data(), yb.size() * 2, hipMemcpyHostToDevice));
            L.xofs = dxo; L.xalpha = dxa; L.yofs = dyo; L.ybeta = dyb;
            L.xchunk = nullptr; L.ytab = nullptr;
            std::vector<uint32_t> xc, yt;
            if (orb_plan_resize(P, l, xo, xa, yo, yb, xc, yt)) {
                uint32_t *dxc, *dyt;
                if ((rc = dev_alloc(e, &dxc, xc.size()))) return rc;
                if ((rc = dev_alloc(e, &dyt, yt.size()))) return rc;
                HIP_TRY(hipMemcpy(dxc, xc.data(), xc.size() * 4, hipMemcpyHostToDevice));
                HIP_TRY(hipMemcpy(dyt, yt.data(), yt.size() * 4, hipMemcpyHostToDevice));
                L.xchunk = dxc; L.ytab = dyt;
            }
        }
    }
    e->d_level0 = P.lv[0].img; e->level0_pitch = P.lv[0].img_pitch; e->level0_frame_stride = P.lv[0].img_frame_stride;
    if (bm_ok) {
        uint4 *dth, *dtv;
        if ((rc = dev_alloc(e, &dth, bm_th.size() / 16))) return rc;
        if ((rc = dev_alloc(e, &dtv, bm_tv.size() / 16))) return rc;
        HIP_TRY(hipMemcpy(dth, bm_th.data(), bm_th.size(), hipMemcpyHostToDevice));
        HIP_TRY(hipMemcpy(dtv, bm_tv.data(), bm_tv.size(), hipMemcpyHostToDevice));
        P.bm_th = dth; P.bm_tv = dtv;
    }
    P.desc_blocks_cap = getenv("ORBHIP_TUNE_DESC_BLOCKS") ? atoi(getenv("ORBHIP_TUNE_DESC_BLOCKS")) : 0;
    orbhip_blur_half_widths(P.blur_hw);
    if ((rc = dev_alloc(e, &P.cell_count, B * cells))) return rc;
    if ((rc = dev_alloc(e, &P.cell_list, B * P.cell_list_frame_stride))) return rc;
    if ((rc = dev_alloc(e, &P.keys, B * keys))) return rc;
    if ((rc = dev_alloc(e, &P.node_of, B * keys))) return rc;
    if ((rc = dev_alloc(e, &P.lvl_kp, B * kps))) return rc;
    if ((rc = dev_alloc(e, &P.lvl_perm, B * kps))) return rc;
    if ((rc = dev_alloc(e, &P.lvl_wkey, B * kps))) return rc;
    if ((rc = dev_alloc(e, &P.lvl_angle, B * kps))) return rc;
    if ((rc = dev_alloc(e, &P.lvl_desc, B * kps * 32))) return rc;
    if ((rc = dev_alloc(e, &P.lvl_count, B * e->nlevels))) return rc;
    if ((rc = dev_alloc(e, &P.lvl_ncand, B * e->nlevels))) return rc;
    if ((rc = dev_alloc(e, &P.status, 1))) return rc;
    {
        auto up = [](size_t v) { return (v + 255) & ~(size_t)255; };
        e->ob_kp = up(8 * B); e->ob_desc = e->ob_kp + up(sizeof(orbhip_keypoint) * B * P.max_kp);
        e->outblob_bytes = e->ob_desc + up((size_t)32 * B * P.max_kp);
        if ((rc = dev_alloc(e, &e->d_outblob, e->outblob_bytes))) return rc;
        P.out_count = reinterpret_cast<int32_t *>(e->d_outblob); P.out_mono = P.out_count + B;
        P.out_kp = reinterpret_cast<orbhip_keypoint *>(e->d_outblob + e->ob_kp); P.out_desc = e->d_outblob + e->ob_desc;
    }
    HIP_TRY(hipMemset(P.status, 0, sizeof(int32_t)));
    P.oct_nc = orb_octree_nc(P);
    if (orb_octree_lds_bytes(P.oct_nc) > 150 * 1024) { g_last_error = "per-level quota (or nIni) too large for the LDS-resident octree"; return ORBHIP_E_BADARG; }
    for (int k = 0; k < 3; k++)
        if ((rc = orb_lds_optin(orb_octree_func(k), e->ctx->device, orb_octree_lds_bytes(P.oct_nc)))) return rc;
    e->oct_dmax_tab = orb_octree_dmax(P);
    P.oct_dmax = getenv("ORBHIP_OCTREE") && !strcmp(getenv("ORBHIP_OCTREE"), "iterative") ? 0 : e->oct_dmax_tab;
    if ((rc = orb_lds_optin(orb_fast_cells_func(e->F.small_cells), e->ctx->device, sizeof(uint32_t) * (size_t)e->F.wave_dw))) return rc;
    if (e->F.use_runs && (rc = orb_lds_optin(orb_fast_runs_func(orb_fast_runs_nld(e->F)), e->ctx->device, sizeof(uint32_t) * (size_t)e->F.run_dw))) return rc;
    e->width = width; e->height = height; e->max_batch = max_batch;
    return ORBHIP_OK;
}

int orb_stereo_max_kp();
int orb_stereo_lds_optin(int device, int max_kp);

extern "C" int orbhip_compute_stereo_matches_device(orbhip_extractor *left, orbhip_extractor *right, float mb, float mbf,
                                                    float *d_u_right, float *d_depth, int32_t *d_n_matches)
{
    if (!left || !right || !d_u_right || !d_depth || !(mb > 0) || !(mbf > 0)) return ORBHIP_E_BADARG;
    if (left->P.max_kp > orb_stereo_max_kp() || right->P.max_kp > orb_stereo_max_kp()) {
        g_last_error = "stereo: max_keypoints " + std::to_string(std::max(left->P.max_kp, right->P.max_kp)) + " exceeds " + std::to_string(orb_stereo_max_kp()) +
                       ", the keys the median filter can hold in 160 KB of LDS";
        return ORBHIP_E_BADARG;
    }
    if (!left->max_batch || !right->max_batch || left->last_batch <= 0 || left->last_batch != right->last_batch ||
        left->width != right->width || left->height != right->height || left->nlevels != right->nlevels ||
        left->scale_factor != right->scale_factor || left->P.max_kp != right->P.max_kp) {
        g_last_error = "stereo: extractors must share geometry, feature budget and batch, and have extracted";
        return ORBHIP_E_BADARG;
    }
    HIP_TRY(hipSetDevice(left->ctx->device));
    {
        const int rc = orb_stereo_lds_optin(left->ctx->device, left->P.max_kp);
        if (rc) return rc;
    }
    if (!left->d_stereo_sad) {
        int rc = dev_alloc(left, &left->d_stereo_sad, (size_t)left->max_batch * left->P.max_kp);
        if (rc) return rc;
    }
    if (right->ctx->stream != left->ctx->stream) {
        hipEvent_t ev;
        HIP_TRY(hipEventCreateWithFlags(&ev, hipEventDisableTiming));
        HIP_TRY(hipEventRecord(ev, right->ctx->stream));
        HIP_TRY(hipStreamWaitEvent(left->ctx->stream, ev, 0));
        HIP_TRY(hipEventDestroy(ev));
    }
    StereoArgs A;
    memset(&A, 0, sizeof(A));
    for (int l = 0; l < left->nlevels; l++) {
        const OrbLevel &a = left->P.lv[l], &b = right->P.lv[l];
        A.lv[l].imgL = a.img; A.lv[l].imgR = b.img; A.lv[l].fsL = a.img_frame_stride; A.lv[l].fsR = b.img_frame_stride;
        A.lv[l].pitchL = a.img_pitch; A.lv[l].pitchR = b.img_pitch; A.lv[l].wR = b.w;
        A.lv[l].scale = left->scale[l]; A.lv[l].inv_scale = left->inv_scale[l];
    }
    A.nlevels = left->nlevels; A.batch = left->last_batch; A.max_kp = left->P.max_kp; A.rows0 = left->height;
    A.kpL = left->P.out_kp; A.kpR = right->P.out_kp; A.descL = left->P.out_desc; A.descR = right->P.out_desc;
    A.nL = left->P.out_count; A.nR = right->P.out_count;
    A.mb = mb; A.mbf = mbf; A.u_right = d_u_right; A.depth = d_depth; A.sad = left->d_stereo_sad; A.n_kept = d_n_matches;
    orb_launch_stereo(A, left->ctx->stream);
    HIP_TRY(hipGetLastError());
    if (right->ctx->stream != left->ctx->stream) {
        hipEvent_t ev;
        HIP_TRY(hipEventCreateWithFlags(&ev, hipEventDisableTiming));
        HIP_TRY(hipEventRecord(ev, left->ctx->stream));
        HIP_TRY(hipStreamWaitEvent(right->ctx->stream, ev, 0));
        HIP_TRY(hipEventDestroy(ev));
    }
    return ORBHIP_OK;
}

extern "C" int orbhip_compute_stereo_matches_host(orbhip_extractor *left, orbhip_extractor *right, float mb, float mbf,
                                                  float *u_right_out, float *depth_out, int n, int32_t *n_matches_out)
{
    if (!left || !right || n < 0 || (n && (!u_right_out || !depth_out))) return ORBHIP_E_BADARG;
    if (n_matches_out) *n_matches_out = 0;
    for (int i = 0; i < n; i++) { u_right_out[i] = -1.0f; depth_out[i] = -1.0f; }
    if (n == 0) return ORBHIP_OK;
    if (left->last_batch <= 0 || n > left->P.max_kp) { g_last_error = "stereo: the left extractor holds no extraction of that many keypoints"; return ORBHIP_E_BADARG; }
    const size_t slots = (size_t)left->max_batch * left->P.max_kp;
    uint8_t *w = (uint8_t *)orbhip_ctx_work_internal(left->ctx, 8 * slots + 4 * (size_t)left->max_batch + 256);
    if (!w) return ORBHIP_E_HIP;
    float *d_ur = (float *)w, *d_dp = d_ur + slots;
    int32_t *d_nk = (int32_t *)(d_dp + slots);
    const int rc = orbhip_compute_stereo_matches_device(left, right, mb, mbf, d_ur, d_dp, d_nk);
    if (rc) return rc;
    uint8_t *h = (uint8_t *)orbhip_ctx_pinned_internal(left->ctx, 8 * (size_t)n + 16);
    if (!h) return ORBHIP_E_HIP;
    hipStream_t st = left->ctx->stream;
    HIP_TRY(hipMemcpyAsync(h, d_ur, 4 * (size_t)n, hipMemcpyDeviceToHost, st));
    HIP_TRY(hipMemcpyAsync(h + 4 * (size_t)n, d_dp, 4 * (size_t)n, hipMemcpyDeviceToHost, st));
    HIP_TRY(hipMemcpyAsync(h + 8 * (size_t)n, d_nk, 4, hipMemcpyDeviceToHost, st));
    HIP_TRY(hipStreamSynchronize(st));
    memcpy(u_right_out, h, 4 * (size_t)n); memcpy(depth_out, h + 4 * (size_t)n, 4 * (size_t)n);
    if (n_matches_out) memcpy(n_matches_out, h + 8 * (size_t)n, 4);
    return ORBHIP_OK;
}

extern "C" int orbhip_compute_stereo_fisheye_matches_host(orbhip_extractor *left, orbhip_extractor *right, int cam1_type, const float *cam1,
        int cam2_type, const float *cam2, const float *Rlr, const float *tlr, const float *level_sigma2, int nlevels,
        int32_t *l2r_out, float *depth_out, float *x3d_out, int n_left, int32_t *r2l_out, int n_right, int32_t *n_matches_out)
{
    if (!left || !right || n_left < 0 || n_right < 0 || (n_left && (!l2r_out || !depth_out || !x3d_out)) || (n_right && !r2l_out)) return ORBHIP_E_BADARG;
    if (n_matches_out) *n_matches_out = 0;
    for (int i = 0; i < n_left; i++) { l2r_out[i] = -1; depth_out[i] = -1.0f; x3d_out[3 * i] = x3d_out[3 * i + 1] = x3d_out[3 * i + 2] = 0.0f; }
    for (int i = 0; i < n_right; i++) r2l_out[i] = -1;
    if (n_left == 0) return ORBHIP_OK;
    const orbhip_keypoint *dk, *hk; const uint8_t *dd, *hd; int32_t cl = -1, cr = -1;
    if (orbhip_extractor_last_frame(left, 0, &dk, &dd, &hk, &hd, &cl, nullptr) != ORBHIP_OK || cl != n_left ||
        orbhip_extractor_last_frame(right, 0, &dk, &dd, &hk, &hd, &cr, nullptr) != ORBHIP_OK || cr != n_right) {
        g_last_error = "stereo fisheye: n_left / n_right are not the counts of the extractors' latest host extractions";
        return ORBHIP_E_BADARG;
    }
    if (left->ctx->device != right->ctx->device) { g_last_error = "stereo fisheye: extractors on two devices"; return ORBHIP_E_BADARG; }
    HIP_TRY(hipSetDevice(left->ctx->device));
    const int max_n = std::max(n_left, n_right);
    const size_t words = 6 * (size_t)max_n + 1;
    int32_t *w = (int32_t *)orbhip_ctx_work_internal(left->ctx, 4 * words + 256);
    if (!w) return ORBHIP_E_HIP;
    int32_t *d_l2r = w, *d_r2l = w + max_n, *d_nm = w + 6 * (size_t)max_n;
    float *d_dp = (float *)(w + 2 * (size_t)max_n), *d_x = (float *)(w + 3 * (size_t)max_n);
    hipStream_t st = left->ctx->stream;
    if (right->ctx->stream != st) {
        hipEvent_t ev;
        HIP_TRY(hipEventCreateWithFlags(&ev, hipEventDisableTiming));
        HIP_TRY(hipEventRecord(ev, right->ctx->stream));
        HIP_TRY(hipStreamWaitEvent(st, ev, 0));
        HIP_TRY(hipEventDestroy(ev));
    }
    const int rc = orbhip_compute_stereo_fisheye_matches_device(left->ctx, left->P.out_kp, left->P.out_desc, left->P.out_count, left->P.out_mono,
                                                                 left->P.max_kp, right->P.out_kp, right->P.out_desc, right->P.out_count,
                                                                 right->P.out_mono, right->P.max_kp, 1, max_n, cam1_type, cam1, cam2_type, cam2, Rlr,
                                                                 tlr, level_sigma2, nlevels, d_l2r, d_r2l, d_dp, d_x, d_nm);
    if (rc) return rc;
    if (right->ctx->stream != st) {
        hipEvent_t ev;
        HIP_TRY(hipEventCreateWithFlags(&ev, hipEventDisableTiming));
        HIP_TRY(hipEventRecord(ev, st));
        HIP_TRY(hipStreamWaitEvent(right->ctx->stream, ev, 0));
        HIP_TRY(hipEventDestroy(ev));
    }
    int32_t *h = (int32_t *)orbhip_ctx_pinned_internal(left->ctx, 4 * words + 16);
    if (!h) return ORBHIP_E_HIP;
    HIP_TRY(hipMemcpyAsync(h, w, 4 * words, hipMemcpyDeviceToHost, st));
    HIP_TRY(hipStreamSynchronize(st));
    memcpy(l2r_out, h, 4 * (size_t)n_left);
    if (n_right) memcpy(r2l_out, h + max_n, 4 * (size_t)n_right);
    memcpy(depth_out, h + 2 * (size_t)max_n, 4 * (size_t)n_left);
    memcpy(x3d_out, h + 3 * (size_t)max_n, 12 * (size_t)n_left);
    if (n_matches_out) *n_matches_out = h[6 * (size_t)max_n];
    return ORBHIP_OK;
}

extern "C" int orbhip_extractor_blur_kernel(const orbhip_extractor *e, int batch)
{
    if (!e || !e->max_batch) return -1;
    return orb_blur_kernel(e->P, batch);
}

extern "C" int orbhip_extractor_fast_kernel(const orbhip_extractor *e)
{
    if (!e || !e->max_batch) return -1;
    return orb_fast_variant(e->F);
}

extern "C" int orbhip_extractor_blur_tiled(const orbhip_extractor *e, int batch)
{
    if (!e || !e->max_batch) return -1;
    return e->P.blur_tiled_ok && orb_blur_kernel(e->P, batch) == 2 ? 1 : 0;
}

extern "C" int orbhip_extractor_resize_band_rows(const orbhip_extractor *e, int level)
{
    if (!e || !e->max_batch || level < 1 || level >= e->nlevels) return -1;
    return e->P.lv[level].xchunk ? e->P.lv[level].rs_rows : 0;
}

extern "C" int orbhip_extractor_set_profiling(orbhip_extractor *e, int enable)
{
    if (!e) return ORBHIP_E_BADARG;
    if (enable && !e->ev_created) {
        for (auto &slot : e->ev) for (auto &ev : slot) HIP_TRY(hipEventCreate(&ev));
        e->ev_created = true;
    }
    e->profiling = enable != 0;
    e->ev_calls = 0;
    return ORBHIP_OK;
}

extern "C" int orbhip_extractor_stage_ms(orbhip_extractor *e, float *ms_out)
{
    if (!e || !ms_out || !e->ev_created || e->ev_calls <= 0) return ORBHIP_E_BADARG;
    const int n = std::min(e->ev_calls, ORBHIP_PROF_SLOTS);
    for (int i = 0; i < ORBHIP_STAGE_COUNT; i++) ms_out[i] = 0.f;
    for (int c = 0; c < n; c++) {
        const int slot = (e->ev_calls - 1 - c) % ORBHIP_PROF_SLOTS;
        HIP_TRY(hipEventSynchronize(e->ev[slot][ORBHIP_STAGE_COUNT]));
        for (int i = 0; i < ORBHIP_STAGE_COUNT; i++) {
            float ms = 0.f;
            HIP_TRY(hipEventElapsedTime(&ms, e->ev[slot][i], e->ev[slot][i + 1]));
            ms_out[i] += ms / n;
        }
    }
    e->ev_calls = 0;
    return ORBHIP_OK;
}

static int tune_int(const char *name, int dflt) { const char *v = getenv(name); return v ? atoi(v) : dflt; }

static int run_pipeline(orbhip_extractor *e, int batch, int lap0, int lap1)
{
    OrbParams &P = e->P;
    P.batch = batch; P.lap0 = lap0; P.lap1 = lap1; P.n_cus = e->ctx->n_cus;
    P.blur_tiled = orbhip_extractor_blur_tiled(e, batch) == 1;
    hipStream_t s = e->ctx->stream;
    const bool prof = e->profiling;
    const int slot = e->ev_calls % ORBHIP_PROF_SLOTS;
#define STAGE_MARK(i) do { if (prof) HIP_TRY(hipEventRecord(e->ev[slot][i], s)); } while (0)
    const bool fork = e->overlap && !prof && batch >= ORB_OVERLAP_MIN_BATCH;
    if (fork && !e->aux_ok) {
        HIP_TRY(hipStreamCreateWithFlags(&e->aux, hipStreamNonBlocking));
        HIP_TRY(hipEventCreateWithFlags(&e->ev_fork, hipEventDisableTiming));
        HIP_TRY(hipEventCreateWithFlags(&e->ev_join, hipEventDisableTiming));
        HIP_TRY(hipEventCreateWithFlags(&e->ev_pyr, hipEventDisableTiming));
        e->aux_ok = true;
    }
    FastParams &F = e->F;
    for (int l = 0; l < e->nlevels; l++) { F.lv[l].img = P.lv[l].img; F.lv[l].frame_stride = P.lv[l].img_frame_stride; F.lv[l].img_pitch = P.lv[l].img_pitch; }
    F.batch = batch; F.n_cus = e->ctx->n_cus; F.cell_count = P.cell_count; F.cell_list = P.cell_list; F.cell_list_frame_stride = P.cell_list_frame_stride; F.status = P.status;
    const bool rows = orb_blur_kernel(P, batch) != 0;
    const int fast_waves = fork ? tune_int("ORBHIP_TUNE_FAST_WAVES", rows ? 18 : 10) : 0;
    STAGE_MARK(ORBHIP_STAGE_PYRAMID);
    if (fork && e->nlevels > 1 && rows && tune_int("ORBHIP_TUNE_L0_EARLY", 0)) {
        HIP_TRY(hipEventRecord(e->ev_fork, s));
        HIP_TRY(hipStreamWaitEvent(e->aux, e->ev_fork, 0));
        orb_launch_fast_cells(F, s, fast_waves, 0, 1);
        for (int l = 1; l < e->nlevels; l++) orb_launch_resize(P, l, e->aux);
        HIP_TRY(hipEventRecord(e->ev_pyr, e->aux));
        HIP_TRY(hipStreamWaitEvent(s, e->ev_pyr, 0));
        orb_launch_fast_cells(F, s, fast_waves, 1, e->nlevels);
        orb_launch_blur(P, e->aux, 5);
        HIP_TRY(hipEventRecord(e->ev_join, e->aux));
    } else {
        for (int l = 1; l < e->nlevels; l++) orb_launch_resize(P, l, s);
        STAGE_MARK(ORBHIP_STAGE_FAST_CELLS);
        if (fork) {
            HIP_TRY(hipEventRecord(e->ev_fork, s));
            HIP_TRY(hipStreamWaitEvent(e->aux, e->ev_fork, 0));
        }
        orb_launch_fast_cells(F, s, fast_waves);
        if (fork) {
            if (!tune_int("ORBHIP_TUNE_SKIP_BLUR", 0))
                orb_launch_blur(P, e->aux, tune_int("ORBHIP_TUNE_BLUR_WGS", 5));
            HIP_TRY(hipEventRecord(e->ev_join, e->aux));
        }
    }
    STAGE_MARK(ORBHIP_STAGE_BLUR);
    if (!fork) orb_launch_blur(P, s, 8);
    STAGE_MARK(ORBHIP_STAGE_OCTREE);
    orb_launch_octree(P, s);
    STAGE_MARK(ORBHIP_STAGE_DESC);
    if (fork) HIP_TRY(hipStreamWaitEvent(s, e->ev_join, 0));
    orb_launch_orient_desc(P, s);
    STAGE_MARK(ORBHIP_STAGE_ASSEMBLE);
    orb_launch_assemble(P, s);
    STAGE_MARK(ORBHIP_STAGE_COUNT);
#undef STAGE_MARK
    if (prof) e->ev_calls++;
    HIP_TRY(hipGetLastError());
    e->last_batch = batch;
    e->generation++;
    return ORBHIP_OK;
}

static int run_pipeline_graph(orbhip_extractor *e, int width, int height, int batch, int lap0, int lap1)
{
    if (!(e->graph_valid && e->g_w == width && e->g_h == height && e->g_batch == batch && e->g_lap0 == lap0 && e->g_lap1 == lap1)) {
        if (e->graph_valid) { (void)hipGraphExecDestroy(e->graph_exec); e->graph_valid = false; }
        hipGraph_t graph = nullptr;
        HIP_TRY(hipStreamBeginCapture(e->ctx->stream, hipStreamCaptureModeThreadLocal));
        const int rc = run_pipeline(e, batch, lap0, lap1);
        hipError_t ce = hipStreamEndCapture(e->ctx->stream, &graph);
        if (rc) { if (graph) (void)hipGraphDestroy(graph); return rc; }
        if (ce != hipSuccess) { g_last_error = std::string("hipStreamEndCapture: ") + hipGetErrorString(ce); return ORBHIP_E_HIP; }
        hipError_t ie = hipGraphInstantiate(&e->graph_exec, graph, nullptr, nullptr, 0);
        (void)hipGraphDestroy(graph);
        if (ie != hipSuccess) { g_last_error = std::string("hipGraphInstantiate: ") + hipGetErrorString(ie); return ORBHIP_E_HIP; }
        e->graph_valid = true; e->g_w = width; e->g_h = height; e->g_batch = batch; e->g_lap0 = lap0; e->g_lap1 = lap1;
    }
    HIP_TRY(hipGraphLaunch(e->graph_exec, e->ctx->stream));
    e->last_batch = batch;
    e->generation++;
    return ORBHIP_OK;
}

extern "C" int orbhip_extract_batch_device(orbhip_extractor *e, const uint8_t *d_images, int width, int height,
                                           size_t row_stride, size_t frame_stride, int batch, int lap0, int lap1)
{
    if (!e || batch <= 0 || row_stride < (size_t)width) return ORBHIP_E_BADARG;
    if (!d_images || width <= 0 || height <= 0) return ORBHIP_E_EMPTY;
    HIP_TRY(hipSetDevice(e->ctx->device));
    int rc = orbhip_extractor_reserve(e, width, height, batch);
    if (rc) return rc;
    OrbLevel &L0 = e->P.lv[0];
    const bool aligned = ((uintptr_t)d_images % 4 == 0) && (row_stride % 4 == 0) && (frame_stride % 4 == 0);
    const bool use_graph = e->graph_mode && !e->profiling;
    if (aligned && !use_graph) {
        L0.img = const_cast<uint8_t *>(d_images);
        L0.img_pitch = (int)row_stride;
        L0.img_frame_stride = frame_stride;
    } else {
        L0.img = e->d_level0; L0.img_pitch = e->level0_pitch; L0.img_frame_stride = e->level0_frame_stride;
        for (int f = 0; f < batch; f++)
            HIP_TRY(hipMemcpy2DAsync(L0.img + (size_t)f * L0.img_frame_stride, L0.img_pitch, d_images + (size_t)f * frame_stride,
                                     row_stride, width, height, hipMemcpyDeviceToDevice, e->ctx->stream));
    }
    return use_graph ? run_pipeline_graph(e, width, height, batch, lap0, lap1) : run_pipeline(e, batch, lap0, lap1);
}

extern "C" int orbhip_extractor_set_graph_mode(orbhip_extractor *e, int enable)
{
    if (!e) return ORBHIP_E_BADARG;
    e->graph_mode = enable != 0;
    if (!e->graph_mode && e->graph_valid) { (void)hipGraphExecDestroy(e->graph_exec); e->graph_valid = false; }
    return ORBHIP_OK;
}

extern "C" int orbhip_extractor_results(orbhip_extractor *e, orbhip_keypoint **d_kp, uint8_t **d_desc,
                                        int32_t **d_count, int32_t **d_mono)
{
    if (!e || !e->max_batch) return ORBHIP_E_BADARG;
    if (d_kp) *d_kp = e->P.out_kp;
    if (d_desc) *d_desc = e->P.out_desc;
    if (d_count) *d_count = e->P.out_count;
    if (d_mono) *d_mono = e->P.out_mono;
    return ORBHIP_OK;
}

static int extract_host_core(orbhip_extractor *e, const uint8_t *h_images, int width, int height, size_t row_stride, size_t frame_stride,
                             int batch, int lap0, int lap1)
{
    if (!e || batch <= 0) return ORBHIP_E_BADARG;
    if (!h_images || width <= 0 || height <= 0) return ORBHIP_E_EMPTY;
    if (row_stride < (size_t)width) return ORBHIP_E_BADARG;
    HIP_TRY(hipSetDevice(e->ctx->device));
    int rc = orbhip_extractor_reserve(e, width, height, batch);
    if (rc) return rc;
    hipStream_t s = e->ctx->stream;
    OrbLevel &L0 = e->P.lv[0];
    L0.img = e->d_level0; L0.img_pitch = e->level0_pitch; L0.img_frame_stride = e->level0_frame_stride;
    const size_t in_bytes = (size_t)batch * L0.img_frame_stride;
    if (e->h_in_bytes < in_bytes) {
        if (e->h_in) (void)hipHostFree(e->h_in);
        e->h_in = nullptr; e->h_in_bytes = 0;
        HIP_TRY(hipHostMalloc((void **)&e->h_in, (size_t)e->max_batch * L0.img_frame_stride, hipHostMallocDefault));
        e->h_in_bytes = (size_t)e->max_batch * L0.img_frame_stride;
    }
    if (!e->h_out) HIP_TRY(hipHostMalloc((void **)&e->h_out, e->outblob_bytes, hipHostMallocDefault));
    if (!e->h_status) HIP_TRY(hipHostMalloc((void **)&e->h_status, 256, hipHostMallocDefault));
    for (int f = 0; f < batch; f++) {
        const uint8_t *src = h_images + (size_t)f * frame_stride;
        uint8_t *dst = e->h_in + (size_t)f * L0.img_frame_stride;
        if (row_stride == (size_t)L0.img_pitch) memcpy(dst, src, (size_t)L0.img_pitch * (height - 1) + width);
        else for (int y = 0; y < height; y++) memcpy(dst + (size_t)y * L0.img_pitch, src + (size_t)y * row_stride, width);
    }
    HIP_TRY(hipMemcpyAsync(L0.img, e->h_in, in_bytes, hipMemcpyHostToDevice, s));
    e->view_generation = ~0ull;
    rc = (e->graph_mode && !e->profiling) ? run_pipeline_graph(e, width, height, batch, lap0, lap1) : run_pipeline(e, batch, lap0, lap1);
    if (rc) return rc;
    const size_t B = (size_t)e->max_batch, mk = (size_t)e->P.max_kp;
    if ((size_t)batch == B) HIP_TRY(hipMemcpyAsync(e->h_out, e->d_outblob, e->outblob_bytes, hipMemcpyDeviceToHost, s));
    else {
        HIP_TRY(hipMemcpyAsync(e->h_out, e->d_outblob, 8 * B, hipMemcpyDeviceToHost, s));
        HIP_TRY(hipMemcpyAsync(e->h_out + e->ob_kp, e->d_outblob + e->ob_kp, sizeof(orbhip_keypoint) * mk * batch, hipMemcpyDeviceToHost, s));
        HIP_TRY(hipMemcpyAsync(e->h_out + e->ob_desc, e->d_outblob + e->ob_desc, 32 * mk * batch, hipMemcpyDeviceToHost, s));
    }
    HIP_TRY(hipMemcpyAsync(e->h_status, e->P.status, sizeof(int32_t), hipMemcpyDeviceToHost, s));
    HIP_TRY(hipStreamSynchronize(s));
    if (*e->h_status) {
        g_last_error = "device-side list capacity exceeded";
        (void)hipMemsetAsync(e->P.status, 0, sizeof(int32_t), s);
        return *e->h_status;
    }
    e->view_generation = e->generation;
    return ORBHIP_OK;
}

extern "C" int orbhip_extract_batch_host(orbhip_extractor *e, const uint8_t *h_images, int width, int height,
                                         size_t row_stride, size_t frame_stride, int batch, int lap0, int lap1,
                                         orbhip_keypoint *kp_out, uint8_t *desc_out, int cap,
                                         int32_t *count_out, int32_t *mono_out)
{
    if (e && batch > 0 && h_images && width > 0 && height > 0 && (!kp_out || !desc_out || !count_out || !mono_out)) return ORBHIP_E_BADARG;
    const int rc = extract_host_core(e, h_images, width, height, row_stride, frame_stride, batch, lap0, lap1);
    if (rc) return rc;
    const int32_t *cnt = reinterpret_cast<const int32_t *>(e->h_out), *mono = cnt + e->max_batch;
    const size_t mk = (size_t)e->P.max_kp;
    for (int f = 0; f < batch; f++) {
        count_out[f] = cnt[f]; mono_out[f] = mono[f];
        if (cnt[f] > cap) return ORBHIP_E_CAPACITY;
        if (cnt[f] == 0) continue;
        memcpy(kp_out + (size_t)f * cap, e->h_out + e->ob_kp + sizeof(orbhip_keypoint) * mk * f, sizeof(orbhip_keypoint) * cnt[f]);
        memcpy(desc_out + (size_t)f * cap * 32, e->h_out + e->ob_desc + 32 * mk * f, (size_t)32 * cnt[f]);
    }
    return ORBHIP_OK;
}

extern "C" int orbhip_extract_batch_host_view(orbhip_extractor *e, const uint8_t *h_images, int width, int height, size_t row_stride,
                                              size_t frame_stride, int batch, int lap0, int lap1, const orbhip_keypoint **kp_view,
                                              const uint8_t **desc_view, int *row_capacity, const int32_t **count_view, const int32_t **mono_view)
{
    if (e && batch > 0 && h_images && width > 0 && height > 0 && (!kp_view || !desc_view || !row_capacity || !count_view || !mono_view)) return ORBHIP_E_BADARG;
    const int rc = extract_host_core(e, h_images, width, height, row_stride, frame_stride, batch, lap0, lap1);
    if (rc) return rc;
    *kp_view = reinterpret_cast<const orbhip_keypoint *>(e->h_out + e->ob_kp); *desc_view = e->h_out + e->ob_desc; *row_capacity = e->P.max_kp;
    *count_view = reinterpret_cast<const int32_t *>(e->h_out); *mono_view = *count_view + e->max_batch;
    return ORBHIP_OK;
}

extern "C" int orbhip_extractor_last_frame(orbhip_extractor *e, int frame, const orbhip_keypoint **d_kp, const uint8_t **d_desc,
                                           const orbhip_keypoint **h_kp_view, const uint8_t **h_desc_view, int32_t *count, unsigned long long *generation)
{
    if (!e || !e->max_batch || frame < 0 || frame >= e->last_batch || e->view_generation != e->generation) return ORBHIP_E_BADARG;
    const size_t mk = (size_t)e->P.max_kp;
    if (d_kp) *d_kp = e->P.out_kp + mk * frame;
    if (d_desc) *d_desc = e->P.out_desc + 32 * mk * frame;
    if (h_kp_view) *h_kp_view = reinterpret_cast<const orbhip_keypoint *>(e->h_out + e->ob_kp) + mk * frame;
    if (h_desc_view) *h_desc_view = e->h_out + e->ob_desc + 32 * mk * frame;
    if (count) *count = reinterpret_cast<const int32_t *>(e->h_out)[frame];
    if (generation) *generation = e->generation;
    return ORBHIP_OK;
}

extern "C" int orbhip_extractor_desc_plan(const orbhip_extractor *e, int batch, int32_t *kp_base, int32_t *kp_cap, int32_t *waves_per_xcd)
{
    if (!e || !e->max_batch || batch < 1 || batch > e->max_batch) return ORBHIP_E_BADARG;
    for (int l = 0; l < e->nlevels; l++) { kp_base[l] = e->P.lv[l].kp_base; kp_cap[l] = e->P.lv[l].kp_cap; }
    OrbParams P = e->P;
    P.batch = batch;
    *waves_per_xcd = 2 * orb_orient_desc_blocks(P);
    return ORBHIP_OK;
}

extern "C" int orbhip_extractor_level_dims(const orbhip_extractor *e, int level, int *w, int *h)
{
    if (!e || level < 0 || level >= e->nlevels || !e->max_batch) return ORBHIP_E_BADARG;
    *w = e->P.lv[level].w; *h = e->P.lv[level].h;
    return ORBHIP_OK;
}

static inline int reflect101_host(int p, int n)
{
    if (n == 1) return 0;
    while (p < 0 || p >= n) { if (p < 0) p = -p; else p = 2 * n - 2 - p; }
    return p;
}

extern "C" int orbhip_extractor_get_pyramid_level(orbhip_extractor *e, int frame, int level, int padded,
                                                  uint8_t *h_out, size_t out_stride)
{
    if (!e || !h_out || level < 0 || level >= e->nlevels || frame < 0 || frame >= e->last_batch) return ORBHIP_E_BADARG;
    const OrbLevel &L = e->P.lv[level];
    HIP_TRY(hipSetDevice(e->ctx->device));
    HIP_TRY(hipStreamSynchronize(e->ctx->stream));
    if (!padded) {
        HIP_TRY(hipMemcpy2D(h_out, out_stride, L.img + (size_t)frame * L.img_frame_stride, L.img_pitch, L.w, L.h, hipMemcpyDeviceToHost));
        return ORBHIP_OK;
    }
    std::vector<uint8_t> tmp((size_t)L.w * L.h);
    HIP_TRY(hipMemcpy2D(tmp.data(), L.w, L.img + (size_t)frame * L.img_frame_stride, L.img_pitch, L.w, L.h, hipMemcpyDeviceToHost));
    const int pw = L.w + 2 * ORB_EDGE, ph = L.h + 2 * ORB_EDGE;
    for (int y = 0; y < ph; y++) {
        const uint8_t *srow = tmp.data() + (size_t)reflect101_host(y - ORB_EDGE, L.h) * L.w;
        uint8_t *drow = h_out + (size_t)y * out_stride;
        for (int x = 0; x < pw; x++) drow[x] = srow[reflect101_host(x - ORB_EDGE, L.w)];
    }
    return ORBHIP_OK;
}

extern "C" int orbhip_extractor_get_pyramid_padded(orbhip_extractor *e, int frame, uint8_t *const *levels_out, const size_t *strides)
{
    if (!e || !levels_out || !strides || frame < 0 || frame >= e->last_batch) return ORBHIP_E_BADARG;
    HIP_TRY(hipSetDevice(e->ctx->device));
    hipStream_t s = e->ctx->stream;
    size_t total = 0;
    for (int l = 0; l < e->nlevels; l++) {
        const OrbLevel &L = e->P.lv[l];
        if (!levels_out[l] || strides[l] < (size_t)L.w + 2 * ORB_EDGE) return ORBHIP_E_BADARG;
        total += ((size_t)L.img_pitch * L.h + 255) & ~(size_t)255;
    }
    if (e->h_pyr_bytes < total) {
        if (e->h_pyr) (void)hipHostFree(e->h_pyr);
        e->h_pyr = nullptr; e->h_pyr_bytes = 0;
        HIP_TRY(hipHostMalloc((void **)&e->h_pyr, total, hipHostMallocDefault));
        e->h_pyr_bytes = total;
    }
    size_t off = 0;
    for (int l = 0; l < e->nlevels; l++) {
        const OrbLevel &L = e->P.lv[l];
        HIP_TRY(hipMemcpyAsync(e->h_pyr + off, L.img + (size_t)frame * L.img_frame_stride, (size_t)L.img_pitch * (L.h - 1) + L.w, hipMemcpyDeviceToHost, s));
        off += ((size_t)L.img_pitch * L.h + 255) & ~(size_t)255;
    }
    HIP_TRY(hipStreamSynchronize(s));
    off = 0;
    for (int l = 0; l < e->nlevels; l++) {
        const OrbLevel &L = e->P.lv[l];
        for (int y = 0; y < L.h; y++) memcpy(levels_out[l] + (size_t)(y + ORB_EDGE) * strides[l] + ORB_EDGE, e->h_pyr + off + (size_t)y * L.img_pitch, L.w);
        off += ((size_t)L.img_pitch * L.h + 255) & ~(size_t)255;
    }
    for (int l = 0; l < e->nlevels; l++) {
        const OrbLevel &L = e->P.lv[l];
        const size_t st = strides[l];
        uint8_t *base = levels_out[l];
        for (int y = ORB_EDGE; y < L.h + ORB_EDGE; y++) {
            uint8_t *row = base + (size_t)y * st;
            for (int x = 0; x < ORB_EDGE; x++) {
                row[x] = row[ORB_EDGE + reflect101_host(x - ORB_EDGE, L.w)];
                row[L.w + ORB_EDGE + x] = row[ORB_EDGE + reflect101_host(L.w + x, L.w)];
            }
        }
        for (int y = 0; y < ORB_EDGE; y++) {
            memcpy(base + (size_t)y * st, base + (size_t)(ORB_EDGE + reflect101_host(y - ORB_EDGE, L.h)) * st, (size_t)L.w + 2 * ORB_EDGE);
            memcpy(base + (size_t)(L.h + ORB_EDGE + y) * st, base + (size_t)(ORB_EDGE + reflect101_host(L.h + y, L.h)) * st, (size_t)L.w + 2 * ORB_EDGE);
        }
    }
    return ORBHIP_OK;
}

extern "C" int orbhip_extractor_get_blurred_level(orbhip_extractor *e, int frame, int level, uint8_t *h_out, size_t out_stride)
{
    if (!e || !h_out || level < 0 || level >= e->nlevels || frame < 0 || frame >= e->last_batch) return ORBHIP_E_BADARG;
    const OrbLevel &L = e->P.lv[level];
    HIP_TRY(hipSetDevice(e->ctx->device));
    HIP_TRY(hipStreamSynchronize(e->ctx->stream));
    if (orbhip_extractor_blur_tiled(e, e->last_batch) == 1) {
        const int tiles_x = L.blur_tiles_x, tiles_y = (L.h + 7) / 8;
        std::vector<uint8_t> t((size_t)tiles_x * tiles_y * 128);
        HIP_TRY(hipMemcpy(t.data(), L.blur + (size_t)frame * L.blur_frame_stride, t.size(), hipMemcpyDeviceToHost));
        for (int y = 0; y < L.h; y++)
            for (int x = 0; x < L.w; x += 16)
                memcpy(h_out + (size_t)y * out_stride + x, t.data() + ORB_BLUR_TILE_OFF(x, y, tiles_x), (size_t)std::min(16, L.w - x));
        return ORBHIP_OK;
    }
    HIP_TRY(hipMemcpy2D(h_out, out_stride, L.blur + (size_t)frame * L.blur_frame_stride, L.blur_pitch, L.w, L.h, hipMemcpyDeviceToHost));
    return ORBHIP_OK;
}

extern "C" int orbhip_extractor_get_fast_candidates(orbhip_extractor *e, int frame, int level, int32_t *xs, int32_t *ys,
                                                    int32_t *scores, int cap, int32_t *n_out)
{
    if (!e || level < 0 || level >= e->nlevels || frame < 0 || frame >= e->last_batch || !n_out) return ORBHIP_E_BADARG;
    const OrbParams &P = e->P;
    const OrbLevel &L = P.lv[level];
    HIP_TRY(hipSetDevice(e->ctx->device));
    HIP_TRY(hipStreamSynchronize(e->ctx->stream));
    int32_t n = 0;
    HIP_TRY(hipMemcpy(&n, P.lvl_ncand + frame * P.nlevels + level, sizeof(n), hipMemcpyDeviceToHost));
    *n_out = n;
    int m = std::min(n, cap);
    if (m > 0 && xs && ys && scores) {
        std::vector<uint32_t> k(m);
        HIP_TRY(hipMemcpy(k.data(), P.keys + (size_t)frame * P.keys_per_frame + L.key_base, sizeof(uint32_t) * m, hipMemcpyDeviceToHost));
        for (int i = 0; i < m; i++) { xs[i] = ORB_KEY_X(k[i]); ys[i] = ORB_KEY_Y(k[i]); scores[i] = ORB_KEY_S(k[i]); }
    }
    return ORBHIP_OK;
}

extern "C" int orbhip_debug_octree(orbhip_extractor *e, int level, int nframes, const int32_t *offs, const int32_t *xs, const int32_t *ys,
                                   const int32_t *scores, int form, uint32_t *out_keys, int cap, int32_t *out_counts, int32_t *out_redo)
{
// ... 74 lines not shown
```

orb-slam3-mac_amd/python/orbhip.py:

```python
import ctypes as C
import os
import numpy as np

try:
    import torch
except Exception:
    torch = None

_HERE = os.path.dirname(os.path.abspath(__file__))
LIB_DIR = os.path.join(os.path.dirname(_HERE), "lib")
LIB_PATH = os.path.join(LIB_DIR, "liborbhip.so")
SYNTH_PATH = os.path.join(LIB_DIR, "libsynth.so")

if not os.path.exists(LIB_PATH):
    raise ImportError(
        "liborbhip.so not built: run `python -c 'import __graft_entry__ as g; g.build()'` "
        "(there is no CPU fallback for the HIP path)")

lib = C.CDLL(LIB_PATH)

OK, E_BADARG, E_NODEVICE, E_HIP, E_CAPACITY, E_ABORTED, E_NOTSPD, E_EMPTY = 0, -1, -2, -3, -4, -5, -6, -7
STAGES = ["pyramid", "fast_cells", "blur", "octree", "desc", "assemble"]

KP_DTYPE = np.dtype([("x", "<f4"), ("y", "<f4"), ("size", "<f4"), ("angle", "<f4"),
                     ("response", "<f4"), ("octave", "<i4"), ("class_id", "<i4")])
assert KP_DTYPE.itemsize == 28

vp, ci, cf, cd, sz = C.c_void_p, C.c_int, C.c_float, C.c_double, C.c_size_t
lib.orbhip_version.restype = C.c_char_p
lib.orbhip_last_error.restype = C.c_char_p
lib.orbhip_ctx_create.argtypes = [ci, vp, C.POINTER(vp)]
lib.orbhip_ctx_destroy.argtypes = [vp]
lib.orbhip_ctx_synchronize.argtypes = [vp]
lib.orbhip_ctx_stream.argtypes = [vp]
lib.orbhip_ctx_stream.restype = vp
lib.orbhip_extractor_create.argtypes = [vp, ci, cf, ci, ci, ci, C.POINTER(vp)]
lib.orbhip_extractor_destroy.argtypes = [vp]
lib.orbhip_extractor_levels.argtypes = [vp]
lib.orbhip_extractor_table.argtypes = [vp, ci, vp]
lib.orbhip_extractor_features_per_level.argtypes = [vp, vp]
lib.orbhip_extractor_umax.argtypes = [vp, vp]
lib.orbhip_blur_half_widths.argtypes = [vp]
lib.orbhip_extractor_reserve.argtypes = [vp, ci, ci, ci]
lib.orbhip_extractor_max_keypoints.argtypes = [vp]
lib.orbhip_extract_batch_device.argtypes = [vp, vp, ci, ci, sz, sz, ci, ci, ci]
lib.orbhip_extractor_results.argtypes = [vp, C.POINTER(vp), C.POINTER(vp), C.POINTER(vp), C.POINTER(vp)]
lib.orbhip_extract_batch_host.argtypes = [vp, vp, ci, ci, sz, sz, ci, ci, ci, vp, vp, ci, vp, vp]
lib.orbhip_extractor_level_dims.argtypes = [vp, ci, C.POINTER(ci), C.POINTER(ci)]
lib.orbhip_extractor_get_pyramid_level.argtypes = [vp, ci, ci, ci, vp, sz]
lib.orbhip_extractor_get_blurred_level.argtypes = [vp, ci, ci, vp, sz]
lib.orbhip_extractor_get_pyramid_padded.argtypes = [vp, ci, vp, vp]
lib.orbhip_extractor_get_fast_candidates.argtypes = [vp, ci, ci, vp, vp, vp, ci, C.POINTER(C.c_int32)]
lib.orbhip_extractor_get_level_keypoints.argtypes = [vp, ci, ci, vp, ci, C.POINTER(C.c_int32)]
lib.orbhip_extractor_set_profiling.argtypes = [vp, ci]
lib.orbhip_extractor_set_graph_mode.argtypes = [vp, ci]
lib.orbhip_extractor_stage_ms.argtypes = [vp, vp]
lib.orbhip_descriptor_distance.argtypes = [vp, vp]
lib.orbhip_match_bf2nn_device.argtypes = [vp, vp, vp, sz, vp, vp, sz, ci, ci, cd, vp, vp, vp]
lib.orbhip_search_for_initialization_device.argtypes = [vp, vp, vp, vp, vp, vp, vp, ci, ci, sz, cf, cf, cf, cf, ci, cf, ci,
                                                        vp, vp, vp]
lib.orbhip_ctx_check_status.argtypes = [vp]
lib.orbhip_ctx_wait_for.argtypes = [vp, vp]
lib.orbhip_extractor_blur_kernel.argtypes = [vp, ci]
lib.orbhip_extractor_blur_kernel.restype = ci
if hasattr(lib, "orbhip_extractor_fast_kernel"):
    lib.orbhip_extractor_fast_kernel.argtypes = [vp]
    lib.orbhip_extractor_fast_kernel.restype = ci
lib.orbhip_extractor_blur_tiled.argtypes = [vp, ci]
lib.orbhip_extractor_blur_tiled.restype = ci
lib.orbhip_extractor_resize_band_rows.argtypes = [vp, ci]
lib.orbhip_extractor_resize_band_rows.restype = ci
if hasattr(lib, "orbhip_extractor_desc_plan"):
    lib.orbhip_extractor_desc_plan.argtypes = [vp, ci, vp, vp, C.POINTER(ci)]
if hasattr(lib, "orbhip_debug_octree"):
    lib.orbhip_debug_octree.argtypes = [vp, ci, ci, vp, vp, vp, vp, ci, vp, ci, vp, vp]
lib.orbhip_prev_matched_init_device.argtypes = [vp, vp, sz, ci, ci, vp]
lib.orbhip_search_by_projection_device.argtypes = [vp, vp, vp, vp, ci, vp, vp, vp, vp, ci, sz, ci, cf, cf, cf, cf, ci, ci, vp, vp]
lib.orbhip_search_local_map_device.argtypes = [vp, vp, vp, vp, ci, vp, vp, vp, vp, ci, sz, ci, cf, cf, cf, cf, ci, cf, vp, vp]


class OrbHipError(RuntimeError):
    def __init__(self, code, where):
        self.code = code
        super().__init__("%s failed: %d (%s)" % (where, code, lib.orbhip_last_error().decode()))


def _chk(rc, where):
    if rc != OK:
        raise OrbHipError(rc, where)


class Context:
    def __init__(self, device=0, stream=None):
        h = vp()
        _chk(lib.orbhip_ctx_create(device, stream, C.byref(h)), "orbhip_ctx_create")
        self.h = h

    def synchronize(self):
        _chk(lib.orbhip_ctx_synchronize(self.h), "orbhip_ctx_synchronize")

    def check_status(self):
        _chk(lib.orbhip_ctx_check_status(self.h), "orbhip_ctx_check_status")

    def wait_for(self, other):
        _chk(lib.orbhip_ctx_wait_for(self.h, other.h), "orbhip_ctx_wait_for")

    @property
    def stream(self):
        return lib.orbhip_ctx_stream(self.h)

    def close(self):
        if self.h:
            lib.orbhip_ctx_destroy(self.h)
            self.h = None


def blur_half_widths():
    out = np.zeros(19, np.int32)
    _chk(lib.orbhip_blur_half_widths(out.ctypes.data), "orbhip_blur_half_widths")
    return out


class Extractor:

    def __init__(self, ctx, nfeatures=1000, scale_factor=1.2, nlevels=8, ini_th=20, min_th=7):
        h = vp()
        _chk(lib.orbhip_extractor_create(ctx.h, nfeatures, scale_factor, nlevels, ini_th, min_th, C.byref(h)),
             "orbhip_extractor_create")
        self.h, self.ctx, self.nlevels = h, ctx, nlevels

    def close(self):
        if self.h:
            lib.orbhip_extractor_destroy(self.h)
            self.h = None

    def table(self, which):
        out = np.zeros(self.nlevels, np.float32)
        _chk(lib.orbhip_extractor_table(self.h, which, out.ctypes.data), "orbhip_extractor_table")
        return out

    def features_per_level(self):
        out = np.zeros(self.nlevels, np.int32)
        _chk(lib.orbhip_extractor_features_per_level(self.h, out.ctypes.data), "features_per_level")
        return out

    def umax(self):
        out = np.zeros(16, np.int32)
        _chk(lib.orbhip_extractor_umax(self.h, out.ctypes.data), "umax")
        return out

    def reserve(self, w, h, batch):
        _chk(lib.orbhip_extractor_reserve(self.h, w, h, batch), "orbhip_extractor_reserve")

    @property
    def max_keypoints(self):
        return lib.orbhip_extractor_max_keypoints(self.h)

    def blur_kernel(self, batch):
        return ("k_blur", "k_blur_rows", "k_blur_mfma")[lib.orbhip_extractor_blur_kernel(self.h, int(batch))]

    def fast_kernel(self):
        return lib.orbhip_extractor_fast_kernel(self.h)

    def blur_tiled(self, batch):
        return lib.orbhip_extractor_blur_tiled(self.h, int(batch)) == 1

    def desc_plan(self, batch):
        base, cap, waves = np.zeros(self.nlevels, np.int32), np.zeros(self.nlevels, np.int32), ci()
        _chk(lib.orbhip_extractor_desc_plan(self.h, int(batch), base.ctypes.data, cap.ctypes.data, C.byref(waves)), "desc_plan")
        return base, cap, waves.value

    def resize_band_rows(self, level):
        return lib.orbhip_extractor_resize_band_rows(self.h, int(level))

    def debug_octree(self, level, lists, form):
        offs = np.zeros(len(lists) + 1, np.int32)
        offs[1:] = np.cumsum([len(l[0]) for l in lists])
        xs, ys, ss = (np.ascontiguousarray(np.concatenate([np.asarray(l[k], np.int32) for l in lists] + [np.zeros(1, np.int32)])) for k in range(3))
        cap = int(max(len(l[0]) for l in lists)) + 16
        keys = np.zeros((len(lists), cap), np.uint32)
        counts, redo = np.zeros(len(lists), np.int32), np.zeros(len(lists), np.int32)
        _chk(lib.orbhip_debug_octree(self.h, int(level), len(lists), offs.ctypes.data, xs.ctypes.data, ys.ctypes.data, ss.ctypes.data,
                                     {"iterative": 0, "table": 1}[form], keys.ctypes.data, cap, counts.ctypes.data, redo.ctypes.data),
             "orbhip_debug_octree")
        kept = [np.stack([k & 0xFFF, (k >> 12) & 0xFFF, k >> 24], 1).astype(np.int32) for k in (keys[f, :counts[f]] for f in range(len(lists)))]
        return kept, redo.tolist()

    def set_graph_mode(self, on):
        _chk(lib.orbhip_extractor_set_graph_mode(self.h, 1 if on else 0), "orbhip_extractor_set_graph_mode")

    def set_profiling(self, on):
        _chk(lib.orbhip_extractor_set_profiling(self.h, 1 if on else 0), "set_profiling")

    def stage_ms(self):
        out = np.zeros(len(STAGES), np.float32)
        _chk(lib.orbhip_extractor_stage_ms(self.h, out.ctypes.data), "stage_ms")
        return dict(zip(STAGES, out.tolist()))

    def extract_host(self, images, lap=(0, 1000)):
        img = np.ascontiguousarray(images, np.uint8)
        if img.ndim == 2:
            img = img[None]
        B, H, W = img.shape
        self.reserve(W, H, B)
        cap = self.max_keypoints
        kp = np.zeros((B, cap), KP_DTYPE)
        desc = np.zeros((B, cap, 32), np.uint8)
        cnt = np.zeros(B, np.int32)
        mono = np.zeros(B, np.int32)
        _chk(lib.orbhip_extract_batch_host(self.h, img.ctypes.data, W, H, W, W * H, B, lap[0], lap[1],
                                           kp.ctypes.data, desc.ctypes.data, cap, cnt.ctypes.data, mono.ctypes.data),
             "orbhip_extract_batch_host")
        return [(kp[f, :cnt[f]].copy(), desc[f, :cnt[f]].copy(), int(mono[f])) for f in range(B)]

    def extract_device(self, d_ptr, w, h, row_stride, frame_stride, batch, lap=(0, 1000)):
        _chk(lib.orbhip_extract_batch_device(self.h, d_ptr, w, h, row_stride, frame_stride, batch, lap[0], lap[1]),
             "orbhip_extract_batch_device")

    def results_device(self):
        a, b, c, d = vp(), vp(), vp(), vp()
        _chk(lib.orbhip_extractor_results(self.h, C.byref(a), C.byref(b), C.byref(c), C.byref(d)), "results")
        return a.value, b.value, c.value, d.value

    def level_dims(self, level):
        w, h = ci(), ci()
        _chk(lib.orbhip_extractor_level_dims(self.h, level, C.byref(w), C.byref(h)), "level_dims")
        return w.value, h.value

    def pyramid_level(self, frame, level, padded=False):
        w, h = self.level_dims(level)
        if padded:
            w, h = w + 38, h + 38
        out = np.zeros((h, w), np.uint8)
        _chk(lib.orbhip_extractor_get_pyramid_level(self.h, frame, level, 1 if padded else 0, out.ctypes.data, w),
             "get_pyramid_level")
        return out

    def pyramid_padded(self, frame):
        outs = [np.zeros((h + 38, w + 38), np.uint8) for w, h in (self.level_dims(l) for l in range(self.nlevels))]
        ptrs = (vp * self.nlevels)(*[o.ctypes.data for o in outs])
        strides = (C.c_size_t * self.nlevels)(*[o.shape[1] for o in outs])
        _chk(lib.orbhip_extractor_get_pyramid_padded(self.h, frame, ptrs, strides), "get_pyramid_padded")
        return outs

    def blurred_level(self, frame, level):
        w, h = self.level_dims(level)
        out = np.zeros((h, w), np.uint8)
        _chk(lib.orbhip_extractor_get_blurred_level(self.h, frame, level, out.ctypes.data, w), "get_blurred_level")
        return out

    def fast_candidates(self, frame, level, cap=1 << 17):
        xs, ys, ss = (np.zeros(cap, np.int32) for _ in range(3))
        n = C.c_int32()
        _chk(lib.orbhip_extractor_get_fast_candidates(self.h, frame, level, xs.ctypes.data, ys.ctypes.data,
                                                      ss.ctypes.data, cap, C.byref(n)), "get_fast_candidates")
        return xs[:n.value].copy(), ys[:n.value].copy(), ss[:n.value].copy()

    def level_keypoints(self, frame, level, cap=8192):
        out = np.zeros(cap, KP_DTYPE)
        n = C.c_int32()
        _chk(lib.orbhip_extractor_get_level_keypoints(self.h, frame, level, out.ctypes.data, cap, C.byref(n)),
             "get_level_keypoints")
        return out[:n.value].copy()


def match_bf2nn_device(ctx, d_descA, d_nA, strideA, d_descB, d_nB, strideB, pairs, max_n, ratio, d_idx2, d_dist2,
                       d_accept):
    _chk(lib.orbhip_match_bf2nn_device(ctx.h, d_descA, d_nA, strideA, d_descB, d_nB, strideB, pairs, max_n, ratio,
                                       d_idx2, d_dist2, d_accept), "orbhip_match_bf2nn_device")


def search_for_initialization_device(ctx, d_kpA, d_descA, d_nA, d_kpB, d_descB, d_nB, pairs, max_n, kp_stride, bounds,
                                     window, nn_ratio, check_ori, d_prev, d_m12, d_nmatches):
    _chk(lib.orbhip_search_for_initialization_device(ctx.h, d_kpA, d_descA, d_nA, d_kpB, d_descB, d_nB, pairs, max_n,
                                                     kp_stride, bounds[0], bounds[1], bounds[2], bounds[3], window,
                                                     nn_ratio, 1 if check_ori else 0, d_prev, d_m12, d_nmatches),
         "orbhip_search_for_initialization_device")


PROJ_QUERY_DTYPE = np.dtype([("u", np.float32), ("v", np.float32), ("radius", np.float32), ("ur", np.float32),
                             ("angle", np.float32), ("min_level", np.int32), ("max_level", np.int32), ("has_obs", np.int32)])


def search_by_projection_device(ctx, d_q, d_desc_q, d_nq, max_q, d_kp, d_desc, d_u_right, d_n, max_n, kp_stride, pairs,
                                bounds, th_high, check_ori, d_train_match, d_nmatches):
    _chk(lib.orbhip_search_by_projection_device(ctx.h, d_q, d_desc_q, d_nq, max_q, d_kp, d_desc, d_u_right, d_n, max_n,
                                                kp_stride, pairs, bounds[0], bounds[1], bounds[2], bounds[3], th_high,
                                                1 if check_ori else 0, d_train_match, d_nmatches),
         "orbhip_search_by_projection_device")


def search_local_map_device(ctx, d_q, d_desc_q, d_nq, max_q, d_kp, d_desc, d_u_right, d_n, max_n, kp_stride, pairs,
                            bounds, th_high, nn_ratio, d_train_match, d_nmatches):
    _chk(lib.orbhip_search_local_map_device(ctx.h, d_q, d_desc_q, d_nq, max_q, d_kp, d_desc, d_u_right, d_n, max_n,
                                            kp_stride, pairs, bounds[0], bounds[1], bounds[2], bounds[3], th_high,
                                            nn_ratio, d_train_match, d_nmatches), "orbhip_search_local_map_device")


lib.orbhip_debug_sbp_handed_back.argtypes = [vp, vp, ci, vp]


def debug_sbp_handed_back(ctx, cap=1 << 16):
    flags = np.zeros(max(cap, 1), np.int32); pairs = C.c_int(0)
    _chk(lib.orbhip_debug_sbp_handed_back(ctx.h, flags.ctypes.data, cap, C.byref(pairs)), "orbhip_debug_sbp_handed_back")
    return flags[:min(pairs.value, cap)].copy()


def prev_matched_init_device(ctx, d_kp, kp_stride, frames, max_n, d_prev):
    _chk(lib.orbhip_prev_matched_init_device(ctx.h, d_kp, kp_stride, frames, max_n, d_prev), "orbhip_prev_matched_init_device")


def descriptor_distance(a, b):
    a = np.ascontiguousarray(a, np.uint8)
    b = np.ascontiguousarray(b, np.uint8)
    return lib.orbhip_descriptor_distance(a.ctypes.data, b.ctypes.data)


_synth = None


def synth_lib():
    global _synth
    if _synth is None:
        _synth = C.CDLL(SYNTH_PATH)
        _synth.synth_frame.argtypes = [vp, ci, ci, ci, C.c_uint64, ci]
        _synth.synth_batch.argtypes = [vp, ci, ci, ci, C.c_uint64, ci]
        _synth.synth_frame_transform.argtypes = [C.c_uint64, ci, C.POINTER(cf), C.POINTER(cf), C.POINTER(cf)]
    return _synth


def synth_frames(w, h, n, seed=20241004, first=0):
    out = np.zeros((n, h, w), np.uint8)
    synth_lib().synth_batch(out.ctypes.data, w, h, n, seed, first)
    return out


def rig2_fields(g):
    r = g.get("rig2")
    if r is None:
        return ((cd * 7)(0, 0, 0, 0, 0, 0, 0), 0.0, 0.0, 0.0, 0.0, 0, (cd * 4)(0, 0, 0, 0))
    kb2 = r.get("kb")
    return ((cd * 7)(*r["Trl"]), *[float(c) for c in r["cam"]], 1 if kb2 is not None else 0, (cd * 4)(*(kb2 if kb2 is not None else (0, 0, 0, 0))))


class BaCamera(C.Structure):
    _fields_ = [("fx", cd), ("fy", cd), ("cx", cd), ("cy", cd), ("bf", cd), ("camera_model", C.c_int32), ("kb", cd * 4),
                ("Trl", cd * 7), ("fx2", cd), ("fy2", cd), ("cx2", cd), ("cy2", cd), ("camera2_model", C.c_int32), ("kb2", cd * 4)]


class BaGraph(C.Structure):
    _fields_ = [("n_poses", C.c_int32), ("n_points", C.c_int32), ("n_edges", C.c_int32),
                ("pose_fixed", vp), ("edge_pose", vp), ("edge_point", vp), ("edge_obs", vp),
                ("edge_inv_sigma2", vp), ("edge_stereo", vp),
                ("fx", cd), ("fy", cd), ("cx", cd), ("cy", cd), ("bf", cd),
                ("camera_model", C.c_int32), ("kb", cd * 4),
                ("Trl", cd * 7), ("fx2", cd), ("fy2", cd), ("cx2", cd), ("cy2", cd), ("camera2_model", C.c_int32), ("kb2", cd * 4),
                ("n_cameras", C.c_int32), ("cameras", vp), ("pose_camera", vp)]


def camera_table(g, cls=None):
    cls = cls or BaCamera
    cams = g.get("cameras")
    if not cams:
        return 0, None, None
    arr = (cls * len(cams))()
    for i, c in enumerate(cams):
        kb = c.get("kb")
        arr[i] = cls(c["fx"], c["fy"], c["cx"], c["cy"], c["bf"], 1 if kb is not None else 0, (cd * 4)(*(kb if kb is not None else (0, 0, 0, 0))),
                     *rig2_fields(dict(rig2=c.get("rig2"))))
    return len(cams), arr, np.ascontiguousarray(g["pose_camera"], np.int32)


class BaParams(C.Structure):
    _fields_ = [("iters1", C.c_int32), ("iters2", C.c_int32), ("huber_mono2", cd), ("huber_stereo2", cd),
                ("user_lambda_init", cd), ("tau", cd), ("max_trials", C.c_int32),
                ("stage2_exclude_outliers", C.c_int32), ("stage2_drop_robust", C.c_int32), ("no_discard", C.c_int32),
                ("gate_mono2", cd), ("gate_stereo2", cd)]


class BaStats(C.Structure):
    _fields_ = [("iterations_run", C.c_int32 * 2), ("lm_trials", C.c_int32), ("n_outliers", C.c_int32),
                ("discarded", C.c_int32), ("chi2_initial", cd), ("chi2_final", cd)]

    def as_dict(self):
        return dict(iterations_run=list(self.iterations_run), lm_trials=self.lm_trials, n_outliers=self.n_outliers,
                    discarded=self.discarded, chi2_initial=self.chi2_initial, chi2_final=self.chi2_final)


lib.orbhip_ba_default_params.argtypes = [C.POINTER(BaParams)]
lib.orbhip_ba_merge_params.argtypes = [C.POINTER(BaParams)]
lib.orbhip_ba_batch_create.argtypes = [vp, vp, ci, vp, vp, C.POINTER(vp)]
lib.orbhip_ba_batch_solve.argtypes = [vp, C.POINTER(BaParams), vp]
lib.orbhip_ba_batch_download.argtypes = [vp, vp, vp, vp, vp]
lib.orbhip_ba_batch_ticks.argtypes = [vp]
lib.orbhip_ba_batch_destroy.argtypes = [vp]
lib.orbhip_ba_solve_batch.argtypes = [vp, vp, ci, C.POINTER(BaParams), vp, vp, vp, vp, vp]
lib.orbhip_ba_batch_set_profiling.argtypes = [vp, ci]
lib.orbhip_ba_batch_gemm_profile.argtypes = [vp, C.POINTER(cf), C.POINTER(ci), C.POINTER(cd)]
lib.orbhip_mfma_f64_peak_tflops.argtypes = [vp, C.POINTER(cd)]
lib.orbhip_ba_batch_gemm_dense_flops.argtypes = [vp]
lib.orbhip_ba_batch_gemm_issued_flops.argtypes = [vp]
lib.orbhip_ba_batch_gemm_issued_flops.restype = cd
lib.orbhip_ba_batch_gemm_dense_flops.restype = cd


def mfma_f64_peak_tflops(ctx):
    v = cd()
    _chk(lib.orbhip_mfma_f64_peak_tflops(ctx.h, C.byref(v)), "orbhip_mfma_f64_peak_tflops")
    return v.value


lib.orbhip_ctx_set_ba_schur_mode.argtypes = [vp, ci]


def ba_set_schur_mode(ctx, mode):
    _chk(lib.orbhip_ctx_set_ba_schur_mode(ctx.h, mode), "orbhip_ctx_set_ba_schur_mode")


def ba_merge_params():
    p = BaParams()
    lib.orbhip_ba_merge_params(C.byref(p))
    return p


def ba_global_params(iterations, robust=True):
# ... 1070 lines not shown
```

Before: 346,800 frames/s.

## Precompute per-cell FAST geometry table and use 32-bit cell iteration with hop stepping

Moves per-cell geometry (origin, clipped extent, thread split, division magic, key offset, list offset) from device-side decoding into a host-built table. The non-runs FAST cell kernel loads each cell's record through a constant-address-space pointer. It also replaces the 64-bit chunk/decode loop with 32-bit counters and a precomputed hop (quotient/remainder), which avoids per-cell level search and division. The change adds a launch-time overflow check that returns an error for very large batches, and exposes the table through a debug API.

```diff
diff --git a/include/orbhip.h b/include/orbhip.h
--- a/include/orbhip.h
+++ b/include/orbhip.h
@@ -42,6 +42,7 @@
 int orbhip_extractor_features_per_level(const orbhip_extractor *ext, int *out);
 int orbhip_extractor_umax(const orbhip_extractor *ext, int *out16);
 int orbhip_blur_half_widths(int *out19);
+int orbhip_fast_cell_table(int nlevels, const int *w, const int *h, int *out, int cap);
 
 int orbhip_extractor_reserve(orbhip_extractor *ext, int width, int height, int max_batch);
 int orbhip_extractor_max_keypoints(const orbhip_extractor *ext);
diff --git a/orb-slam3-mac_amd/csrc/fast_kernels.hip b/orb-slam3-mac_amd/csrc/fast_kernels.hip
--- a/orb-slam3-mac_amd/csrc/fast_kernels.hip
+++ b/orb-slam3-mac_amd/csrc/fast_kernels.hip
@@ -6,6 +6,7 @@
 #include <cstdio>
 #include <cstdlib>
 #include <cstring>
+#include <cmath>
 
 typedef short s16x2 __attribute__((ext_vector_type(2)));
 typedef uint32_t u32_unaligned __attribute__((aligned(1)));
@@ -98,30 +99,20 @@
     const s16x2 Lc = pkmax3(FC_U(q[-SPITCH - 1]), FC_U(q[-1]), FC_U(q[SPITCH - 1])); \
     const s16x2 Rc = pkmax3(FC_U(q[-SPITCH + 1]), FC_U(q[1]), FC_U(q[SPITCH + 1]))
 
-struct FcCell {
-    int frame, lvl, ci, cj;
-    int dw, dh;
-    int ipitch;
-    const uint8_t *src;
-    int ncols, nrows, wcell, hcell, cell_base, cell_cap, tpr, rpt;
-};
+struct FcSrc { int dh, ipitch; const uint8_t *src; };
 #define FC_SGPR(x) __builtin_amdgcn_readfirstlane(x)
-__device__ __forceinline__ void fc_cell_geom(const FastParams &P, FcCell &C)
-{
-    const FcLevel &L = P.lv[C.lvl];
-    C.ncols = FC_SGPR(L.ncols); C.nrows = FC_SGPR(L.nrows); C.wcell = FC_SGPR(L.wcell); C.hcell = FC_SGPR(L.hcell);
-    C.cell_base = FC_SGPR(L.cell_base); C.cell_cap = FC_SGPR(L.cell_cap); C.tpr = FC_SGPR(L.tpr); C.rpt = FC_SGPR(L.rpt);
-    C.ipitch = FC_SGPR(L.img_pitch) & 0xFFFF;
-    const int max_bx = FC_SGPR(L.max_bx), max_by = FC_SGPR(L.max_by);
-    const int ini_y = ORB_MINB + C.ci * C.hcell, ini_x = ORB_MINB + C.cj * C.wcell;
-    int max_y = ini_y + C.hcell + 6, max_x = ini_x + C.wcell + 6;
-    C.src = L.img + (size_t)C.frame * L.frame_stride + (size_t)(ini_y * C.ipitch + ini_x - 1);
-    C.dw = 0; C.dh = 0;
-    if (ini_y >= max_by - 3 || ini_x >= max_bx - 6) return;
-    if (max_y > max_by) max_y = max_by;
-    if (max_x > max_bx) max_x = max_bx;
-    C.dw = max_x - ini_x - 6; C.dh = max_y - ini_y - 6;
-    if (C.dw <= 0 || C.dh <= 0) { C.dw = 0; C.dh = 0; }
+typedef uint32_t fc_u32x4 __attribute__((ext_vector_type(4)));
+typedef const __attribute__((address_space(4))) fc_u32x4 *fc_tab_ptr;
+__device__ __forceinline__ FcRecord fc_load_record(const FcRecord *tab, int i)
+{
+    const fc_u32x4 v = ((fc_tab_ptr)(uintptr_t)tab)[i];
+    return FcRecord{v.x, v.y, v.z, v.w};
+}
+__device__ __forceinline__ FcSrc fc_cell_src(const FastParams &P, const FcRecord &R, int frame)
+{
+    const FcImage &I = P.im[fc_rec_level(R)];
+    const int ipitch = I.pitch & 0xFFFF;
+    return FcSrc{fc_rec_dh(R), ipitch, I.img + (size_t)(uint32_t)frame * I.frame_stride + (uint32_t)(fc_rec_y0(R) * ipitch + fc_rec_x0(R))};
 }
 template <int NCH, int NLD, typename CELL>
 __device__ __forceinline__ void fc_issue_loads(const CELL &C, int lane, uint4 (&ld)[NLD])
@@ -144,7 +135,7 @@
     if (reset) { unsigned long long z[12] = {0}; if (hipMemcpyToSymbol(HIP_SYMBOL(g_fc_prof), z, 96) != hipSuccess) return -1; }
     return 0;
 }
-#define FC_T(i) do { const unsigned long long t_ = __builtin_readcyclecounter(); fc_acc[i] += t_ - fc_prev; fc_prev = t_; } while (0)
+#define FC_T(i) do { const unsigned long long t_ = __builtin_readcyclecounter(); if (lane == 0) fc_acc[i] += t_ - fc_prev; fc_prev = t_; } while (0)
 #else
 #define FC_T(i) do { } while (0)
 #endif
@@ -158,69 +149,53 @@
     uint16_t *SC = reinterpret_cast<uint16_t *>(PT + P.rows * PITCH);
     uint16_t *Q = SC + (P.srows + 2) * SPITCH;
     const unsigned lid = xcd_logical_id(blockIdx.x, gridDim.x);
-    const int lvl_lo = FC_SGPR(P.lvl_lo), lvl_hi = FC_SGPR(P.lvl_hi);
-    const int cell_lo = FC_SGPR(P.lv[lvl_lo].cell_base);
-    const int cps = (lvl_hi < P.nlevels ? FC_SGPR(P.lv[lvl_hi].cell_base) : FC_SGPR(P.cells_per_frame)) - cell_lo;
-    const long total_cells = (long)P.batch * cps;
-    const int chunk = FC_SGPR(P.chunk);
-    const long nchunks = (total_cells + chunk - 1) / chunk;
-    if ((long)lid >= nchunks) return;
-    const int nlevels = lvl_hi, ini_th = FC_SGPR(P.ini_th), min_th = FC_SGPR(P.min_th), cpf = FC_SGPR(P.cells_per_frame);
-    auto decode = [&](long gi, FcCell &X) {
-        X.frame = (int)(gi / cps);
-        const int cell = cell_lo + (int)(gi - (long)X.frame * cps);
-        X.lvl = lvl_lo;
-        for (int l = lvl_lo + 1; l < nlevels; l++) if (cell >= P.lv[l].cell_base) X.lvl = l;
-        const int c = cell - P.lv[X.lvl].cell_base;
-        X.ci = c / P.lv[X.lvl].ncols; X.cj = c - X.ci * P.lv[X.lvl].ncols;
-        X.frame = FC_SGPR(X.frame); X.lvl = FC_SGPR(X.lvl); X.ci = FC_SGPR(X.ci); X.cj = FC_SGPR(X.cj);
-        fc_cell_geom(P, X);
-    };
-    long ch = lid;
-    long g = ch * chunk, g_end = min(g + chunk, total_cells);
-    FcCell C;
-    decode(g, C);
+    const uint32_t chunk = (uint32_t)FC_SGPR(P.chunk), ncells = FC_SGPR(P.total);
+    uint32_t g = FC_SGPR(lid * chunk);
+    if (g >= ncells) return;
+    const int cell_lo = FC_SGPR(P.cell_lo), cell_hi = FC_SGPR(P.cell_hi), cps = cell_hi - cell_lo;
+    const int ini_th = FC_SGPR(P.ini_th), min_th = FC_SGPR(P.min_th), cpf = FC_SGPR(P.cells_per_frame);
+    int frame = FC_SGPR((int)(g / (uint32_t)cps));
+    int ti = cell_lo + (int)(g - (uint32_t)frame * (uint32_t)cps);
+    uint32_t left = min(chunk, ncells - g) - 1;
+    FcRecord R = fc_load_record(P.cell_tab, ti);
     uint4 ld[NLD];
-    fc_issue_loads<NCH, NLD>(C, lane, ld);
+    fc_issue_loads<NCH, NLD>(fc_cell_src(P, R, frame), lane, ld);
     const int lo_th = min(ini_th, min_th);
 #ifdef FC_PROF
-    unsigned long long fc_acc[12] = {0, 0, 0, 0, 0, 0, 0, 0, 0, 0, 0, 0}, fc_prev = __builtin_readcyclecounter();
+    __shared__ unsigned long long fc_acc[12];
+    if (lane < 12) fc_acc[lane] = 0;
+    unsigned long long fc_prev = __builtin_readcyclecounter();
     const unsigned long long fc_t0 = fc_prev;
 #endif
     for (bool more = true; more;) {
-        const int dw = C.dw, dh = C.dh;
+        const bool inside = left > 0;
+        const uint32_t gn = g + (inside ? 1u : FC_SGPR(P.hop));
+        more = gn < ncells;
+        int nframe = frame + (inside ? 0 : (int)FC_SGPR(P.hop_q)), nti = ti + (inside ? 1 : (int)FC_SGPR(P.hop_r));
+        if (nti >= cell_hi) { nti -= cps; nframe++; }
+        const FcRecord N = fc_load_record(P.cell_tab, more ? nti : ti);
+        left = inside ? left - 1 : min(chunk, ncells - gn) - 1;
+        const int dw = fc_rec_dw(R), dh = fc_rec_dh(R);
         const int npb = (dw + 1) >> 1;
-        const int cell = C.cell_base + C.ci * C.ncols + C.cj;
-        uint32_t *cnt_out = P.cell_count + (size_t)C.frame * cpf + cell;
-        uint32_t *list = P.cell_list + (size_t)C.frame * P.cell_list_frame_stride + (size_t)cell * C.cell_cap;
-        const int key_x0 = 3 + C.cj * C.wcell, key_y0 = 3 + C.ci * C.hcell;
-        const int cell_cap = C.cell_cap, tpr = C.tpr, rptT = C.rpt;
+        uint32_t *cnt_out = P.cell_count + (uint32_t)(frame * cpf + ti);
+        uint32_t *list = P.cell_list + ((size_t)(uint32_t)frame * P.cell_list_frame_stride + R.list);
+        const uint32_t key0 = fc_rec_key0(R);
+        const int cell_cap = FC_SGPR(P.cell_cap), tpr = fc_rec_tpr(R), rptT = fc_rec_rpt(R);
+        const uint32_t magic = fc_rec_magic(R);
 #ifdef FC_PROF
         __builtin_amdgcn_s_waitcnt(0x0F70);
         FC_T(11);
 #endif
         if (dw > 0) FC_STAGE(NCH, NLD);
         FC_T(8);
-        FcCell N = C;
-        g++;
-        if (g < g_end) {
-            N.cj++;
-            if (N.cj == C.ncols) { N.cj = 0; N.ci++; }
-            if (N.ci == C.nrows) { N.ci = 0; N.lvl++; }
-            if (N.lvl == nlevels) { N.lvl = lvl_lo; N.frame++; }
-            fc_cell_geom(P, N);
-        } else {
-            ch += gridDim.x;
-            more = ch < nchunks;
-            if (more) { g = ch * chunk; g_end = min(g + chunk, total_cells); decode(g, N); }
-        }
+        const FcSrc NS = fc_cell_src(P, N, nframe);
         FC_T(9);
-        if (more) fc_issue_loads<NCH, NLD>(N, lane, ld);
+        if (more) fc_issue_loads<NCH, NLD>(NS, lane, ld);
         FC_T(10);
-        if (dw <= 0) { if (lane == 0) *cnt_out = 0; C = N; continue; }
+        if (dw <= 0) { if (lane == 0) *cnt_out = 0; R = N; g = gn; frame = nframe; ti = nti; continue; }
         FC_T(0);
         wave_lds_sync();
-        const int tr0 = (int)(__umul24((uint32_t)lane, P.div_magic[tpr]) >> 16), tg = lane - tr0 * tpr;
+        const int tr0 = (int)(__umul24((uint32_t)lane, magic) >> 16), tg = lane - tr0 * tpr;
         const bool lane_rows = tr0 < rptT && 2 * tg < npb, pair1 = 2 * tg + 1 < npb;
         int total = 0;
         FC_T(1);
@@ -277,8 +252,8 @@
                 const int mine = __popc(keep);
                 const int inc = wave_incl_scan(mine);
                 int offs = total + inc - mine;
-                if (keep & 1u) { if (offs < cell_cap) list[offs] = ORB_PACK_KEY(2 * bp + key_x0, by + key_y0, sc & 0xFFu); offs++; }
-                if (keep & 2u) { if (offs < cell_cap) list[offs] = ORB_PACK_KEY(2 * bp + 1 + key_x0, by + key_y0, (sc >> 8) & 0xFFu); }
+                if (keep & 1u) { if (offs < cell_cap) list[offs] = ORB_PACK_KEY(2 * bp, by, sc & 0xFFu) + key0; offs++; }
+                if (keep & 2u) { if (offs < cell_cap) list[offs] = ORB_PACK_KEY(2 * bp + 1, by, (sc >> 8) & 0xFFu) + key0; }
                 total += __builtin_amdgcn_readlane(inc, 63);
             }
             FC_T(4);
@@ -287,15 +262,16 @@
         }
         if (total > cell_cap) { if (lane == 0) atomicExch(P.status, ORBHIP_E_CAPACITY); total = cell_cap; }
         if (lane == 0) *cnt_out = (uint32_t)total;
-        C = N;
+        R = N; g = gn; frame = nframe; ti = nti;
         FC_T(5);
 #ifdef FC_PROF
-        fc_acc[6]++;
+        if (lane == 0) fc_acc[6]++;
 #endif
     }
 #ifdef FC_PROF
-    fc_acc[7] = __builtin_readcyclecounter() - fc_t0;
-    if (lane == 0) for (int i = 0; i < 12; i++) atomicAdd(&g_fc_prof[i], fc_acc[i]);
+    if (lane == 0) fc_acc[7] = __builtin_readcyclecounter() - fc_t0;
+    wave_lds_sync();
+    if (lane < 12) atomicAdd(&g_fc_prof[lane], fc_acc[lane]);
 #endif
 }
 
@@ -313,11 +289,12 @@
     const FcLevel &L = P.lv[C.lvl];
     C.ncols = FC_SGPR(L.ncols); C.nrows = FC_SGPR(L.nrows); C.wcell = FC_SGPR(L.wcell); C.hcell = FC_SGPR(L.hcell);
     C.cell_base = FC_SGPR(L.cell_base); C.cell_cap = FC_SGPR(L.cell_cap); C.rpc = FC_SGPR(L.rpc); C.rpr = FC_SGPR(L.rpr);
-    C.ipitch = FC_SGPR(L.img_pitch) & 0xFFFF;
+    const FcImage &I = P.im[C.lvl];
+    C.ipitch = FC_SGPR(I.pitch) & 0xFFFF;
     C.nc = min(C.rpc, C.ncols - C.cj);
     const int max_bx = FC_SGPR(L.max_bx), max_by = FC_SGPR(L.max_by);
     const int ini_y = ORB_MINB + C.ci * C.hcell, ini_x = ORB_MINB + C.cj * C.wcell;
-    C.src = L.img + (size_t)C.frame * L.frame_stride + (size_t)(ini_y * C.ipitch + ini_x - 1);
+    C.src = I.img + (size_t)C.frame * I.frame_stride + (size_t)(ini_y * C.ipitch + ini_x - 1);
     C.dw0 = 0; C.dw1 = 0; C.dh = 0;
     if (ini_y >= max_by - 3) return;
     C.dh = min(ini_y + C.hcell + 6, max_by) - ini_y - 6;
@@ -503,9 +480,40 @@
 
 int orb_fast_runs_nld(const FastParams &F) { return (F.run_rows - 7) * FR_NCH <= 256 ? 4 : 6; }
 int orb_fast_variant(const FastParams &F) { return F.use_runs ? (orb_fast_runs_nld(F) == 4 ? 2 : 3) : F.small_cells ? 1 : 0; }
-void orb_plan_fast(const OrbParams &P, FastParams &F)
+bool orb_plan_cell_grid(OrbLevel &L)
+{
+    const float w_ = (float)((L.w - ORB_EDGE + 3) - ORB_MINB), h_ = (float)((L.h - ORB_EDGE + 3) - ORB_MINB);
+    if (w_ < 30.f || h_ < 30.f) return false;
+    L.ncols = (int)(w_ / 30.f); L.nrows = (int)(h_ / 30.f);
+    L.wcell = (int)ceilf(w_ / L.ncols); L.hcell = (int)ceilf(h_ / L.nrows);
+    return true;
+}
+void orb_plan_fast(const OrbParams &P, FastParams &F, std::vector<FcRecord> &cell_tab)
 {
     memset(&F, 0, sizeof(F));
+    cell_tab.clear(); cell_tab.reserve((size_t)P.cells_per_frame);
+    for (int l = 0; l < P.nlevels; l++) {
+        const OrbLevel &L = P.lv[l];
+        const int max_bx = L.w - ORB_MINB, max_by = L.h - ORB_MINB;
+        const int npb = (L.wcell + 1) >> 1;
+        const uint32_t tpr = (uint32_t)((npb + 1) >> 1), magic = 65536u / tpr + 1;
+        for (int ci = 0; ci < L.nrows; ci++)
+            for (int cj = 0; cj < L.ncols; cj++) {
+                const int ini_y = ORB_MINB + ci * L.hcell, ini_x = ORB_MINB + cj * L.wcell;
+                int dw = 0, dh = 0;
+                if (!(ini_y >= max_by - 3 || ini_x >= max_bx - 6)) {
+                    dw = std::min(ini_x + L.wcell + 6, max_bx) - ini_x - 6; dh = std::min(ini_y + L.hcell + 6, max_by) - ini_y - 6;
+                    if (dw <= 0 || dh <= 0) dw = dh = 0;
+                }
+                FcRecord r;
+                r.xy = (uint32_t)(ini_x - 1) | (uint32_t)ini_y << 16;
+                r.band = (uint32_t)dw | (uint32_t)dh << 6 | tpr << 12 | magic << 16;
+                r.key = ORB_PACK_KEY(3 + cj * L.wcell, 3 + ci * L.hcell, l);
+                r.list = (uint32_t)(L.cell_base + ci * L.ncols + cj) * (uint32_t)L.cell_cap;
+                cell_tab.push_back(r);
+            }
+    }
+    F.cell_cap = P.lv[0].cell_cap;
     int mw = 0, mh = 0;
     bool small = true;
     for (int l = 0; l < P.nlevels; l++) {
@@ -515,7 +523,6 @@
         f.max_bx = L.w - ORB_MINB; f.max_by = L.h - ORB_MINB;
         f.ncols = L.ncols; f.nrows = L.nrows; f.wcell = L.wcell; f.hcell = L.hcell; f.cell_base = L.cell_base; f.cell_cap = L.cell_cap;
         const int npb = (L.wcell + 1) >> 1;
-        f.tpr = (npb + 1) >> 1; f.rpt = 64 / f.tpr;
         small = small && npb + 4 <= 24 && npb + 2 <= 24 && (L.hcell + 6) * 3 <= 64 * 2;
     }
     {
@@ -543,14 +550,41 @@
     F.wave_dw = F.rows * (small ? 24 : 40) + ((F.srows + 2) * (small ? 24 : 32) + F.qcap + 1) / 2;
     F.wave_dw = (F.wave_dw + 3) & ~3;
     F.nlevels = P.nlevels; F.ini_th = P.ini_th; F.min_th = P.min_th; F.cells_per_frame = P.cells_per_frame;
-    for (int n = 1; n < 34; n++) F.div_magic[n] = (uint32_t)(65536 / n + 1);
-}
-
-void orb_launch_fast_cells(const FastParams &F_, hipStream_t s, int max_per_cu, int lvl_lo, int lvl_hi)
+}
+extern "C" int orbhip_fast_cell_table(int nlevels, const int *w, const int *h, int *out, int cap)
+{
+    if (nlevels < 1 || nlevels > ORB_MAX_LEVELS || !w || !h || (!out && cap > 0)) return ORBHIP_E_BADARG;
+    OrbParams P;
+    memset(&P, 0, sizeof(P));
+    P.nlevels = nlevels;
+    int cells = 0, cell_cap = 0;
+    for (int l = 0; l < nlevels; l++) {
+        OrbLevel &L = P.lv[l];
+        L.w = w[l]; L.h = h[l];
+        if (!orb_plan_cell_grid(L) || L.wcell + 6 > 64 || L.hcell + 6 > 64) return ORBHIP_E_BADARG;
+        cell_cap = std::max(cell_cap, ((L.wcell + 1) / 2) * ((L.hcell + 1) / 2));
+        L.cell_base = cells; cells += L.ncols * L.nrows;
+    }
+    for (int l = 0; l < nlevels; l++) P.lv[l].cell_cap = cell_cap;
+    P.cells_per_frame = cells;
+    FastParams F;
+    std::vector<FcRecord> tab;
+    orb_plan_fast(P, F, tab);
+    for (int i = 0; i < cells && i < cap; i++) {
+        const FcRecord &r = tab[i];
+        const uint32_t k = fc_rec_key0(r);
+        const int v[12] = {fc_rec_level(r), fc_rec_x0(r), fc_rec_y0(r), fc_rec_dw(r), fc_rec_dh(r), ORB_KEY_X(k), ORB_KEY_Y(k), (int)r.list,
+                           fc_rec_tpr(r), fc_rec_rpt(r), (int)fc_rec_magic(r), F.cell_cap};
+        memcpy(out + 12 * i, v, sizeof(v));
+    }
+    return cells;
+}
+
+bool orb_launch_fast_cells(const FastParams &F_, hipStream_t s, int max_per_cu, int lvl_lo, int lvl_hi)
 {
     FastParams F = F_;
     F.lvl_lo = lvl_lo; F.lvl_hi = lvl_hi < 0 ? F.nlevels : lvl_hi;
-    if (F.lvl_lo >= F.lvl_hi) return;
+    if (F.lvl_lo >= F.lvl_hi) return true;
     const bool runs = F.use_runs != 0;
     const size_t lds = sizeof(uint32_t) * (size_t)(runs ? F.run_dw : F.wave_dw);
     const int nld = orb_fast_runs_nld(F);
@@ -579,10 +613,18 @@
     static const int chunk_env = getenv("ORBHIP_TUNE_FAST_CHUNK") ? atoi(getenv("ORBHIP_TUNE_FAST_CHUNK")) : 0;
     const long fair = total / (8 * nblocks);
     const int cmax = runs ? 8 : 4;
-    F.chunk = chunk_env > 0 ? chunk_env : (int)(fair < 1 ? 1 : fair > cmax ? cmax : fair);
+    F.chunk = chunk_env > 0 ? std::min(chunk_env, 1 << 16) : (int)(fair < 1 ? 1 : fair > cmax ? cmax : fair);
+    if (!runs) {
+        const long hop = nblocks * F.chunk - F.chunk + 1;
+        if (total + nblocks * (long)F.chunk >= (1l << 32) || (long)F.batch * F.cells_per_frame >= (1l << 31)) return false;
+        F.cell_lo = F.lv[F.lvl_lo].cell_base; F.cell_hi = F.lvl_hi < F.nlevels ? F.lv[F.lvl_hi].cell_base : F.cells_per_frame;
+        const long cps = F.cell_hi - F.cell_lo;
+        F.total = (uint32_t)total; F.hop = (uint32_t)hop; F.hop_q = (uint32_t)(hop / cps); F.hop_r = (uint32_t)(hop % cps);
+    }
     if (runs && nld == 4) hipLaunchKernelGGL(k_fast_runs<4>, dim3((unsigned)nblocks), dim3(64), lds, s, F);
     else if (runs) hipLaunchKernelGGL(k_fast_runs<6>, dim3((unsigned)nblocks), dim3(64), lds, s, F);
     else if (F.small_cells) hipLaunchKernelGGL((k_fast_cells<3, 24, 2>), dim3((unsigned)nblocks), dim3(64), lds, s, F);
     else hipLaunchKernelGGL((k_fast_cells<5, 32, 5>), dim3((unsigned)nblocks), dim3(64), lds, s, F);
+    return true;
 }
 const void *orb_fast_cells_func(int small) { return small ? reinterpret_cast<const void *>(k_fast_cells<3, 24, 2>) : reinterpret_cast<const void *>(k_fast_cells<5, 32, 5>); }
diff --git a/orb-slam3-mac_amd/csrc/orb_internal.h b/orb-slam3-mac_amd/csrc/orb_internal.h
--- a/orb-slam3-mac_amd/csrc/orb_internal.h
+++ b/orb-slam3-mac_amd/csrc/orb_internal.h
@@ -80,21 +80,33 @@
 };
 
 struct FcLevel {
-    const uint8_t *img; size_t frame_stride; int img_pitch;
     int max_bx, max_by;
     int ncols, nrows, wcell, hcell, cell_base, cell_cap;
-    int tpr, rpt;
     int rpc, rpr, run_base;
 };
+struct FcImage { const uint8_t *img; size_t frame_stride; int pitch, pad_; };
+struct FcRecord { uint32_t xy, band, key, list; };
+__host__ __device__ __forceinline__ int fc_rec_x0(const FcRecord &r) { return (int)(r.xy & 0xFFFFu); }
+__host__ __device__ __forceinline__ int fc_rec_y0(const FcRecord &r) { return (int)(r.xy >> 16); }
+__host__ __device__ __forceinline__ int fc_rec_dw(const FcRecord &r) { return (int)(r.band & 63u); }
+__host__ __device__ __forceinline__ int fc_rec_dh(const FcRecord &r) { return (int)((r.band >> 6) & 63u); }
+__host__ __device__ __forceinline__ int fc_rec_tpr(const FcRecord &r) { return (int)((r.band >> 12) & 15u); }
+__host__ __device__ __forceinline__ uint32_t fc_rec_magic(const FcRecord &r) { return r.band >> 16; }
+__host__ __device__ __forceinline__ int fc_rec_rpt(const FcRecord &r) { return (int)(r.band >> 26); }
+__host__ __device__ __forceinline__ uint32_t fc_rec_key0(const FcRecord &r) { return r.key & 0xFFFFFFu; }
+__host__ __device__ __forceinline__ int fc_rec_level(const FcRecord &r) { return (int)(r.key >> 24); }
 struct FastParams {
     FcLevel lv[ORB_MAX_LEVELS];
+    FcImage im[ORB_MAX_LEVELS];
+    const FcRecord *cell_tab;
     int nlevels, batch, ini_th, min_th, cells_per_frame;
+    int cell_cap;
     int n_cus;
     int chunk;
     int lvl_lo, lvl_hi;
+    int cell_lo, cell_hi; uint32_t total, hop, hop_q, hop_r;
     uint32_t *cell_count, *cell_list; size_t cell_list_frame_stride; int32_t *status;
     int rows, srows, qcap, wave_dw, small_cells;
-    uint32_t div_magic[34];
     int runs_per_frame, run_rows, run_q0, run_dw, use_runs;
 };
 
@@ -134,14 +146,15 @@
 
 int orb_lds_optin(const void *func, int device, size_t need);
 
-void orb_plan_fast(const OrbParams &P, FastParams &F);
+bool orb_plan_cell_grid(OrbLevel &L);
+void orb_plan_fast(const OrbParams &P, FastParams &F, std::vector<FcRecord> &cell_tab);
 bool orb_plan_resize(OrbParams &P, int level, const std::vector<int16_t> &xofs, const std::vector<int16_t> &xalpha, const std::vector<int16_t> &yofs,
                      const std::vector<int16_t> &ybeta, std::vector<uint32_t> &xchunk, std::vector<uint32_t> &ytab);
 bool orb_plan_blur(OrbParams &P, std::vector<int8_t> &bm_th, std::vector<int8_t> &bm_tv);
 int orb_blur_kernel(const OrbParams &P, int batch);
 
 void orb_launch_resize(const OrbParams &P, int level, hipStream_t s);
-void orb_launch_fast_cells(const FastParams &F, hipStream_t s, int max_per_cu, int lvl_lo = 0, int lvl_hi = -1);
+bool orb_launch_fast_cells(const FastParams &F, hipStream_t s, int max_per_cu, int lvl_lo = 0, int lvl_hi = -1);
 const void *orb_fast_runs_func(int nld);
 int orb_fast_runs_nld(const FastParams &F);
 int orb_fast_variant(const FastParams &F);
diff --git a/orb-slam3-mac_amd/csrc/orbhip_api.hip b/orb-slam3-mac_amd/csrc/orbhip_api.hip
--- a/orb-slam3-mac_amd/csrc/orbhip_api.hip
+++ b/orb-slam3-mac_amd/csrc/orbhip_api.hip
@@ -405,10 +405,7 @@
         OrbLevel &L = P.lv[l];
         L.w = cv_round_f((float)width * e->inv_scale[l]);
         L.h = cv_round_f((float)height * e->inv_scale[l]);
-        const float w_ = (float)((L.w - ORB_EDGE + 3) - ORB_MINB), h_ = (float)((L.h - ORB_EDGE + 3) - ORB_MINB);
-        if (w_ < 30.f || h_ < 30.f) { g_last_error = "pyramid level smaller than one FAST cell"; return ORBHIP_E_BADARG; }
-        L.ncols = (int)(w_ / 30.f); L.nrows = (int)(h_ / 30.f);
-        L.wcell = (int)ceilf(w_ / L.ncols); L.hcell = (int)ceilf(h_ / L.nrows);
+        if (!orb_plan_cell_grid(L)) { g_last_error = "pyramid level smaller than one FAST cell"; return ORBHIP_E_BADARG; }
         if (L.wcell + 6 > 64 || L.hcell + 6 > 64) { g_last_error = "FAST cell exceeds the 64x64 LDS tile"; return ORBHIP_E_BADARG; }
         max_cell_cap = std::max(max_cell_cap, ((L.wcell + 1) / 2) * ((L.hcell + 1) / 2));
         L.cell_base = cells; cells += L.ncols * L.nrows;
@@ -430,7 +427,8 @@
         keys += align_up(L.key_cap, 4);
     }
     P.cells_per_frame = cells; P.keys_per_frame = keys; P.kps_per_frame = kps; P.max_kp = align_up(kps, 8);
-    orb_plan_fast(P, e->F);
+    std::vector<FcRecord> cell_tab;
+    orb_plan_fast(P, e->F, cell_tab);
     P.rows_min_batch = getenv("ORBHIP_ROWS_MIN_BATCH") ? atoi(getenv("ORBHIP_ROWS_MIN_BATCH")) : 16;
     std::vector<int8_t> bm_th, bm_tv;
     const bool bm_ok = orb_plan_blur(P, bm_th, bm_tv);
@@ -480,6 +478,12 @@
         HIP_TRY(hipMemcpy(dtv, bm_tv.data(), bm_tv.size(), hipMemcpyHostToDevice));
         P.bm_th = dth; P.bm_tv = dtv;
     }
+    {
+        FcRecord *dct;
+        if ((rc = dev_alloc(e, &dct, cell_tab.size()))) return rc;
+        HIP_TRY(hipMemcpy(dct, cell_tab.data(), cell_tab.size() * sizeof(FcRecord), hipMemcpyHostToDevice));
+        e->F.cell_tab = dct;
+    }
     P.desc_blocks_cap = getenv("ORBHIP_TUNE_DESC_BLOCKS") ? atoi(getenv("ORBHIP_TUNE_DESC_BLOCKS")) : 0;
     orbhip_blur_half_widths(P.blur_hw);
     if ((rc = dev_alloc(e, &P.cell_count, B * cells))) return rc;
@@ -720,6 +724,7 @@
     const bool prof = e->profiling;
     const int slot = e->ev_calls % ORBHIP_PROF_SLOTS;
 #define STAGE_MARK(i) do { if (prof) HIP_TRY(hipEventRecord(e->ev[slot][i], s)); } while (0)
+#define FAST_TRY(launch) do { if (!(launch)) { g_last_error = "batch * FAST cells exceeds the 32-bit cell counter of k_fast_cells"; return ORBHIP_E_BADARG; } } while (0)
     const bool fork = e->overlap && !prof && batch >= ORB_OVERLAP_MIN_BATCH;
     if (fork && !e->aux_ok) {
         HIP_TRY(hipStreamCreateWithFlags(&e->aux, hipStreamNonBlocking));
@@ -729,7 +734,7 @@
         e->aux_ok = true;
     }
     FastParams &F = e->F;
-    for (int l = 0; l < e->nlevels; l++) { F.lv[l].img = P.lv[l].img; F.lv[l].frame_stride = P.lv[l].img_frame_stride; F.lv[l].img_pitch = P.lv[l].img_pitch; }
+    for (int l = 0; l < e->nlevels; l++) { F.im[l].img = P.lv[l].img; F.im[l].frame_stride = P.lv[l].img_frame_stride; F.im[l].pitch = P.lv[l].img_pitch; }
     F.batch = batch; F.n_cus = e->ctx->n_cus; F.cell_count = P.cell_count; F.cell_list = P.cell_list; F.cell_list_frame_stride = P.cell_list_frame_stride; F.status = P.status;
     const bool rows = orb_blur_kernel(P, batch) != 0;
     const int fast_waves = fork ? tune_int("ORBHIP_TUNE_FAST_WAVES", rows ? 18 : 10) : 0;
@@ -737,11 +742,11 @@
     if (fork && e->nlevels > 1 && rows && tune_int("ORBHIP_TUNE_L0_EARLY", 0)) {
         HIP_TRY(hipEventRecord(e->ev_fork, s));
         HIP_TRY(hipStreamWaitEvent(e->aux, e->ev_fork, 0));
-        orb_launch_fast_cells(F, s, fast_waves, 0, 1);
+        FAST_TRY(orb_launch_fast_cells(F, s, fast_waves, 0, 1));
         for (int l = 1; l < e->nlevels; l++) orb_launch_resize(P, l, e->aux);
         HIP_TRY(hipEventRecord(e->ev_pyr, e->aux));
         HIP_TRY(hipStreamWaitEvent(s, e->ev_pyr, 0));
-        orb_launch_fast_cells(F, s, fast_waves, 1, e->nlevels);
+        FAST_TRY(orb_launch_fast_cells(F, s, fast_waves, 1, e->nlevels));
         orb_launch_blur(P, e->aux, 5);
         HIP_TRY(hipEventRecord(e->ev_join, e->aux));
     } else {
@@ -751,7 +756,7 @@
             HIP_TRY(hipEventRecord(e->ev_fork, s));
             HIP_TRY(hipStreamWaitEvent(e->aux, e->ev_fork, 0));
         }
-        orb_launch_fast_cells(F, s, fast_waves);
+        FAST_TRY(orb_launch_fast_cells(F, s, fast_waves));
         if (fork) {
             if (!tune_int("ORBHIP_TUNE_SKIP_BLUR", 0))
                 orb_launch_blur(P, e->aux, tune_int("ORBHIP_TUNE_BLUR_WGS", 5));
@@ -769,6 +774,7 @@
     orb_launch_assemble(P, s);
     STAGE_MARK(ORBHIP_STAGE_COUNT);
 #undef STAGE_MARK
+#undef FAST_TRY
     if (prof) e->ev_calls++;
     HIP_TRY(hipGetLastError());
     e->last_batch = batch;
diff --git a/orb-slam3-mac_amd/python/orbhip.py b/orb-slam3-mac_amd/python/orbhip.py
--- a/orb-slam3-mac_amd/python/orbhip.py
+++ b/orb-slam3-mac_amd/python/orbhip.py
@@ -41,6 +41,7 @@
 lib.orbhip_extractor_features_per_level.argtypes = [vp, vp]
 lib.orbhip_extractor_umax.argtypes = [vp, vp]
 lib.orbhip_blur_half_widths.argtypes = [vp]
+lib.orbhip_fast_cell_table.argtypes = [C.c_int, vp, vp, vp, C.c_int]
 lib.orbhip_extractor_reserve.argtypes = [vp, ci, ci, ci]
 lib.orbhip_extractor_max_keypoints.argtypes = [vp]
 lib.orbhip_extract_batch_device.argtypes = [vp, vp, ci, ci, sz, sz, ci, ci, ci]
@@ -121,6 +122,16 @@
     return out
 
 
+def fast_cell_table(widths, heights):
+    w = np.ascontiguousarray(widths, np.int32)
+    h = np.ascontiguousarray(heights, np.int32)
+    n = lib.orbhip_fast_cell_table(len(w), w.ctypes.data, h.ctypes.data, None, 0)
+    _chk(min(n, 0), "orbhip_fast_cell_table")
+    out = np.zeros((n, 12), np.int32)
+    _chk(min(lib.orbhip_fast_cell_table(len(w), w.ctypes.data, h.ctypes.data, out.ctypes.data, n), 0), "orbhip_fast_cell_table")
+    return out
+
+
 class Extractor:
 
     def __init__(self, ctx, nfeatures=1000, scale_factor=1.2, nlevels=8, ini_th=20, min_th=7):
```

Result: faster. 353,200 frames/s, median of 6 (+1.9%).
